# Alibaba-Gemini-Lab/Gemini-SEAL

Measured on AMD Instinct MI355X. Metric: ciphertext multiply+relinearize/s (BFV N=2^15, 8 primes, bit-exact PARITY mode), higher is better.
Workload: dtype u64

## Files before the change

gemini-seal_amd/csrc/devmath.hpp:

```cpp
#pragma once

#include <hip/hip_runtime.h>

#include <cstdint>
#include "ntt_bounds.hpp"
#include "dotacc.hpp"

namespace sealhip
{
    using u64 = unsigned long long;

    struct PrimeDev
    {
        u64 p;
        u64 two_p;
        u64 rdp;
        u64 cr0, cr1;
        u64 inv_n, inv_n_shoup;
        u64 inv_n_w, inv_n_w_shoup;
        u64 ninv;
        const u64 *fwd;
        const u64 *inv;
        const double *fwd_d;
        const double *inv_d;
        double p_d, pinv_d;
    };

    constexpr double kTwo52 = 4503599627370496.0;
    __device__ __forceinline__ double fp_of(u64 bits)
    {
        return __longlong_as_double(static_cast<long long>(bits));
    }
    __device__ __forceinline__ u64 fp_bits(double v)
    {
        return static_cast<u64>(__double_as_longlong(v));
    }
    __device__ __forceinline__ double fp_from_u64(u64 x)
    {
        return fp_of(x | 0x4330000000000000ull) - kTwo52;
    }
    __device__ __forceinline__ u64 fp_to_u64(double r)
    {
        return fp_bits(r + kTwo52) & 0x000FFFFFFFFFFFFFull;
    }
    __device__ __forceinline__ double fp_reduce(double x, double p, double pinv)
    {
#pragma clang fp contract(off)
        return __builtin_fma(-__builtin_rint(x * pinv), p, x);
    }
    __device__ __forceinline__ double fp_canonical(double x, double p, double pinv)
    {
        const double r = fp_reduce(x, p, pinv);
        return r < 0.0 ? r + p : r;
    }
    __device__ __forceinline__ double fp_mulmod(double y, double w, double p, double pinv)
    {
#pragma clang fp contract(off)
        const double h = y * w;
        const double l = __builtin_fma(y, w, -h);
        const double q = __builtin_rint(h * pinv);
        return __builtin_fma(-q, p, h) + l;
    }
    __device__ __forceinline__ void fp_butterfly_fwd(u64 &ub, u64 &yb, u64 wb, double p, double pinv)
    {
        const double u = fp_of(ub), r = fp_mulmod(fp_of(yb), fp_of(wb), p, pinv);
        ub = fp_bits(u + r);
        yb = fp_bits(u - r);
    }
    __device__ __forceinline__ void fp_butterfly_inv(u64 &ub, u64 &yb, u64 wb, double p, double pinv)
    {
        const double u = fp_of(ub), y = fp_of(yb);
        ub = fp_bits(u + y);
        yb = fp_bits(fp_mulmod(u - y, fp_of(wb), p, pinv));
    }

    __device__ __forceinline__ void note_nonzero(unsigned *__restrict__ tflags, std::size_t item, u64 nz)
    {
        if (tflags != nullptr && nz != 0 && tflags[item] == 0)
            tflags[item] = 1;
    }

    __device__ __forceinline__ void store_stream(u64 *p, u64 v)
    {
        __builtin_nontemporal_store(v, p);
    }
    __device__ __forceinline__ void store_stream2(u64 *p, u64 a, u64 b)
    {
        typedef u64 u64x2_s __attribute__((ext_vector_type(2)));
        u64x2_s v;
        v.x = a;
        v.y = b;
        __builtin_nontemporal_store(v, reinterpret_cast<u64x2_s *>(p));
    }

    __device__ __forceinline__ u64 mulhi(u64 a, u64 b)
    {
        return __umul64hi(a, b);
    }

    __device__ __forceinline__ u64 mulmod_lazy(u64 x, u64 y, u64 yshoup, u64 p)
    {
        u64 q = mulhi(x, yshoup);
        return x * y - q * p;
    }

    __device__ __forceinline__ u64 mulmod_shoup(u64 x, u64 y, u64 yshoup, u64 p)
    {
        u64 t = mulmod_lazy(x, y, yshoup, p);
        return t >= p ? t - p : t;
    }

    __device__ __forceinline__ u64 barrett_lazy(u64 x, u64 rdp, u64 p)
    {
        return x - mulhi(x, rdp) * p;
    }

    __device__ __forceinline__ u64 barrett_reduce_128(u64 lo, u64 hi, u64 p, u64 cr0, u64 cr1)
    {
        u64 carry = mulhi(lo, cr0);
        u64 t_lo = lo * cr1, t_hi = mulhi(lo, cr1);
        u64 tmp1 = t_lo + carry;
        u64 tmp3 = t_hi + (tmp1 < t_lo);
        u64 u_lo = hi * cr0, u_hi = mulhi(hi, cr0);
        u64 tmp1b = tmp1 + u_lo;
        u64 carry2 = u_hi + (tmp1b < tmp1);
        u64 q = hi * cr1 + tmp3 + carry2;
        u64 r = lo - q * p;
        return r >= p ? r - p : r;
    }

    __device__ __forceinline__ u64 redc128(u64 lo, u64 hi, u64 p, u64 ninv)
    {
        const u64 m = lo * ninv;
        return hi + mulhi(m, p) + (lo != 0);
    }
    __device__ __forceinline__ u64 redc_finish(u64 t, u64 p, u64 rdp, bool small)
    {
        if (!small)
            t = t - mulhi(t, rdp) * p;
        return t >= p ? t - p : t;
    }

    __device__ __forceinline__ u64 barrett_reduce_63(u64 x, u64 p, u64 cr1)
    {
        u64 r = x - mulhi(x, cr1) * p;
        return r >= p ? r - p : r;
    }

    __device__ __forceinline__ u64 mul_mod(u64 a, u64 b, u64 p, u64 cr0, u64 cr1)
    {
        return barrett_reduce_128(a * b, mulhi(a, b), p, cr0, cr1);
    }

    __device__ __forceinline__ u64 mul_add_mod(u64 a, u64 b, u64 c, u64 p, u64 cr0, u64 cr1)
    {
        u64 lo = a * b, hi = mulhi(a, b);
        u64 lo2 = lo + c;
        hi += (lo2 < lo);
        return barrett_reduce_128(lo2, hi, p, cr0, cr1);
    }

    __device__ __forceinline__ void mac128(u64 &lo, u64 &hi, u64 a, u64 b)
    {
        u64 pl = a * b, ph = mulhi(a, b);
        u64 nl = lo + pl;
        hi += ph + (nl < lo);
        lo = nl;
    }

    __device__ __forceinline__ u64 add_mod(u64 a, u64 b, u64 p)
    {
        u64 s = a + b;
        return s >= p ? s - p : s;
    }
    __device__ __forceinline__ u64 sub_mod(u64 a, u64 b, u64 p)
    {
        u64 d = a - b;
        return a < b ? d + p : d;
// ... 506 lines not shown
```

gemini-seal_amd/csrc/engine.cpp:

```cpp
#include "engine.hpp"

#include <algorithm>
#include <atomic>
#include <cstdlib>
#include <cstring>

namespace sealhip
{
    namespace
    {
        template <class T>
        T *upload(Engine &e, std::vector<void *> &owned, const T *host, std::size_t count)
        {
            T *dev = nullptr;
            SEALHIP_CHECK(hipMalloc(reinterpret_cast<void **>(&dev), sizeof(T) * (count ? count : 1)));
            owned.push_back(dev);
            if (count)
                SEALHIP_CHECK(hipMemcpy(dev, host, sizeof(T) * count, hipMemcpyHostToDevice));
            (void)e;
            return dev;
        }

        RowMap make_map(const std::vector<unsigned short> &ids)
        {
            RowMap m{};
            if (ids.size() > static_cast<std::size_t>(kMaxRows))
                throw std::invalid_argument("too many rows per polynomial");
            m.rows = static_cast<int>(ids.size());
            for (std::size_t i = 0; i < ids.size(); i++)
                m.prime[i] = ids[i];
            return m;
        }
    }

    unsigned long long next_pool_id();

    std::unique_ptr<Engine> make_engine(int scheme, int logn, const u64 *key_moduli, int n_key, int nsp, u64 t,
                                        bool strict, int device)
    {
        if (scheme != 1 && scheme != 2)
            throw std::invalid_argument("unsupported scheme");
        if (logn < 3 || logn > 16)
            throw std::invalid_argument("poly_modulus_degree is invalid");
        if (n_key < 2 || n_key > kMaxModuli || nsp < 1 || n_key <= nsp)
            throw std::invalid_argument("coeff_modulus / n_special_primes invalid");
        if (scheme == 1 && t < 2)
            throw std::invalid_argument("plain_modulus is invalid");
        auto e = std::make_unique<Engine>();
        e->scheme = scheme;
        e->logn = logn;
        e->n = std::size_t(1) << logn;
        e->n_key = n_key;
        e->nsp = nsp;
        e->k_first = n_key - nsp;
        e->t = scheme == 1 ? t : 0;
        e->mode_strict = strict;
        e->use_half_kernel = true;
        e->device = device;
        e->key_moduli.assign(key_moduli, key_moduli + n_key);
        for (int i = 0; i < n_key; i++)
        {
            HostModulus check(e->key_moduli[i]);
            (void)check;
            for (int j = 0; j < i; j++)
                if (e->key_moduli[i] == e->key_moduli[j])
                    throw std::invalid_argument("coeff_modulus primes must be distinct");
        }
        if (scheme == 1)
            e->aux_primes = get_primes(e->n, 60, static_cast<std::size_t>(n_key) + 3);
        const bool batching = scheme == 1 && (t - 1) % (2 * static_cast<u64>(e->n)) == 0 && is_prime_u64(t);
        const int n_primes = n_key + static_cast<int>(e->aux_primes.size()) + (batching ? 1 : 0);
        if (batching)
            e->plain_prime = n_primes - 1;
        e->tables.resize(n_primes);
        for (int i = 0; i < n_primes; i++)
        {
            const u64 p = i == e->plain_prime ? t : i < n_key ? e->key_moduli[i] : e->aux_primes[i - n_key];
            if (i == n_key + 1 && i != e->plain_prime)
            {
                e->tables[i].logn = logn;
                e->tables[i].p = p;
                continue;
            }
            e->tables[i].build(logn, p);
        }
        if (device < 0)
            return e;

        SEALHIP_CHECK(hipSetDevice(device));
        e->lanes = std::make_shared<LanePool>();
        e->lanes->device = device;
        e->lanes->id = next_pool_id();
        SEALHIP_CHECK(ntt_init_kernels());
        std::vector<PrimeDev> pd(n_primes);
        for (int i = 0; i < n_primes; i++)
        {
            const HostNttTables &tb = e->tables[i];
            HostModulus m(tb.p);
            PrimeDev &d = pd[i];
            d.p = tb.p;
            d.two_p = tb.p << 1;
            d.rdp = tb.rdp ? tb.rdp : shoup(1, tb.p);
            d.cr0 = m.cr0;
            d.cr1 = m.cr1;
            d.inv_n = tb.inv_n;
            d.inv_n_shoup = tb.inv_n_shoup;
            d.inv_n_w = tb.inv_n_w;
            d.inv_n_w_shoup = tb.inv_n_w_shoup;
            {
                u64 inv = tb.p;
                for (int it = 0; it < 6; it++)
                    inv *= 2 - tb.p * inv;
                d.ninv = 0 - inv;
            }
            d.fwd = tb.fwd.empty() ? nullptr : upload<u64>(*e, e->owned, tb.fwd.data(), tb.fwd.size());
            d.inv = tb.inv.empty() ? nullptr : upload<u64>(*e, e->owned, tb.inv.data(), tb.inv.size());
            d.fwd_d = d.inv_d = nullptr;
            d.p_d = static_cast<double>(tb.p);
            d.pinv_d = 1.0 / d.p_d;
            if (tb.p < kFpPrimeBound && tb.logn >= 14 && !tb.fwd.empty())
            {
                std::vector<double> f(tb.fwd.size() / 2), v(tb.inv.size() / 2);
                for (std::size_t j = 0; j < f.size(); j++)
                    f[j] = static_cast<double>(tb.fwd[2 * j]);
                for (std::size_t j = 0; j < v.size(); j++)
                    v[j] = static_cast<double>(tb.inv[2 * j]);
                d.fwd_d = upload<double>(*e, e->owned, f.data(), f.size());
                d.inv_d = upload<double>(*e, e->owned, v.data(), v.size());
            }
        }
        e->d_primes = upload<PrimeDev>(*e, e->owned, pd.data(), pd.size());
        return e;
    }

    Lane::~Lane()
    {
        if (device < 0)
            return;
        (void)hipSetDevice(device);
        if (stream)
            (void)hipStreamSynchronize(stream);
        for (ProfRecord &r : prof)
        {
            if (r.start)
                (void)hipEventDestroy(r.start);
            if (r.stop)
                (void)hipEventDestroy(r.stop);
        }
        if (stage)
            free_host_stage(stage);
        if (seed_pin_done)
            (void)hipEventDestroy(seed_pin_done);
        if (seed_pin)
            (void)hipHostFree(seed_pin);
        if (ws)
            (void)hipFree(ws);
        if (d_tickets)
            (void)hipFree(d_tickets);
        if (h_fault)
            (void)hipHostFree(h_fault);
        if (own_stream && stream)
            (void)hipStreamDestroy(stream);
    }

    Lane *LanePool::take()
    {
        std::lock_guard<std::mutex> lock(mu);
        if (!idle.empty())
        {
            Lane *l = idle.back();
            idle.pop_back();
            l->tsink = l->tsink_cur = l->tsink_arm = nullptr;
            l->tsink_cap = l->tsink_base = 0;
            return l;
        }
        auto l = std::make_unique<Lane>();
        l->device = device;
        SEALHIP_CHECK(hipSetDevice(device));
        SEALHIP_CHECK(hipStreamCreateWithFlags(&l->stream, hipStreamNonBlocking));
        l->own_stream = true;
        SEALHIP_CHECK(hipHostMalloc(reinterpret_cast<void **>(&l->h_fault), sizeof(unsigned), hipHostMallocMapped));
        *l->h_fault = 0;
        SEALHIP_CHECK(hipHostGetDevicePointer(reinterpret_cast<void **>(&l->d_fault), l->h_fault, 0));
        all.push_back(std::move(l));
        return all.back().get();
    }

    void LanePool::give(Lane *lane)
    {
        lane->tsink = lane->tsink_cur = lane->tsink_arm = nullptr;
        lane->tsink_cap = lane->tsink_base = 0;
        std::lock_guard<std::mutex> lock(mu);
        idle.push_back(lane);
    }

    namespace
    {
        struct ThreadLanes
        {
            struct Held
            {
                std::weak_ptr<LanePool> pool;
                Lane *lane;
            };
            std::vector<Held> held;
            ~ThreadLanes()
            {
                for (Held &h : held)
                    if (auto p = h.pool.lock())
                        p->give(h.lane);
            }
        };
        thread_local ThreadLanes t_lanes;
        thread_local unsigned long long t_cur_pool_id = 0;
        thread_local Lane *t_cur_lane = nullptr;
        std::atomic<unsigned long long> g_pool_serial{ 0 };
    }

    unsigned long long next_pool_id()
    {
        return ++g_pool_serial;
    }

    Lane &Engine::lane() const
    {
        if (!lanes)
            throw std::logic_error("host-only context: no device");
        if (t_cur_pool_id == lanes->id)
            return *t_cur_lane;
        auto &held = t_lanes.held;
        for (std::size_t i = 0; i < held.size();)
        {
            auto p = held[i].pool.lock();
            if (!p)
            {
                held.erase(held.begin() + static_cast<std::ptrdiff_t>(i));
                continue;
            }
            if (p.get() == lanes.get())
            {
                t_cur_pool_id = lanes->id;
                t_cur_lane = held[i].lane;
                return *t_cur_lane;
            }
            i++;
        }
        Lane *l = lanes->take();
        held.push_back({ lanes, l });
        t_cur_pool_id = lanes->id;
        t_cur_lane = l;
        return *l;
    }

    void Engine::sync_and_check(bool all_lanes) const
    {
        if (all_lanes)
        {
            std::vector<hipStream_t> streams;
            {
                std::lock_guard<std::mutex> lock(lanes->mu);
                for (auto &l : lanes->all)
                    if (!l->capturing)
// ... 790 lines not shown
```

gemini-seal_amd/csrc/engine.hpp:

```cpp
#pragma once

#include <hip/hip_runtime.h>

#include <cstddef>
#include <array>
#include <atomic>
#include <cstdint>
#include <functional>
#include <map>
#include <memory>
#include <mutex>
#include <stdexcept>
#include <string>
#include <cstdlib>
#include <vector>

#include "devmath.hpp"
#include "ntt_bounds.hpp"
#include "hostmath.hpp"

namespace sealhip
{
    constexpr int kMaxRows = 136;
    constexpr int kMaxModuli = 64;
// ... 275 lines not shown
        const std::uint32_t *batch_map();
        mutable std::mutex mu;
        void prof_begin(const char *tag, double units) const;
        void prof_end() const;
        unsigned *ntt_tickets(std::size_t nrows) const;

        ~Engine();
        int n_primes() const
        {
            return static_cast<int>(tables.size());
        }
        LevelTools &level(int k);
        LevelTools &level_host(int k);
        LevelTools &level_rescale(int k);
        const std::uint32_t *galois_table(std::uint32_t elt);
        void ws_reset() const
        {
            Lane &l = lane();
            l.ws_used = l.ws_floor;
        }
        u64 *ws_alloc(std::size_t words) const;
        void ws_reserve(std::size_t bytes) const;
        RowMap map_for(int k, unsigned base);
        int rows_for(int k, unsigned base);
    };

    struct HipError : std::runtime_error
    {
        hipError_t code;
        HipError(hipError_t c, const char *what) : std::runtime_error(what), code(c)
        {}
    };
#define SEALHIP_CHECK(expr)                                                                          \
    do                                                                                               \
    {                                                                                                \
        hipError_t _e = (expr);                                                                      \
        if (_e != hipSuccess)                                                                        \
            throw ::sealhip::HipError(_e, (std::string(#expr) + ": " + hipGetErrorString(_e)).c_str()); \
    } while (0)
    inline void check(hipError_t err, const char *what)
    {
        if (err != hipSuccess)
            throw HipError(err, (std::string(what) + ": " + hipGetErrorString(err)).c_str());
    }

    constexpr int kThreads = 256;
    inline unsigned grid_for(std::size_t work_items, std::size_t max_blocks = 256u * 16u)
    {
        const std::size_t blocks = (work_items + kThreads - 1) / kThreads;
        return static_cast<unsigned>(blocks < max_blocks ? (blocks ? blocks : 1) : max_blocks);
    }

    struct ProfScope
    {
        const Engine &e;
        ProfScope(const Engine &eng, const char *tag, double units) : e(eng)
        {
            if (e.lane().prof_on)
                e.prof_begin(tag, units);
        }
        ~ProfScope()
        {
            if (e.lane().prof_on)
                e.prof_end();
        }
    };

    hipError_t ntt_init_kernels();
    hipError_t ntt_butterfly_rate(const Engine &e, int kind, int prime_id, double *butterflies_per_s);
    hipError_t launch_ntt(const Engine &e, u64 *data, std::size_t nrows, const RowMap &map, bool inverse, int flags);
    bool ntt_can_gather(const Engine &e);
    bool ntt_strict_top_done_ok(const Engine &e, const RowMap &map);
    hipError_t launch_ntt_gather(const Engine &e, u64 *data, std::size_t nrows, const RowMap &map, const NttSource &src,
                                 int flags);

    enum class PolyOp
    {
        Dyadic,
        Add,
        Sub,
        Negate,
        Scalar,
        Mod63
    };
    hipError_t launch_poly_op(const Engine &e, PolyOp op, const u64 *a, const u64 *b, u64 scalar, u64 *r,
                              std::size_t nrows, const RowMap &map);
    hipError_t launch_tensor_product(const Engine &e, const u64 *a, int sa, std::size_t a_stride, const u64 *b, int sb,
                                     std::size_t b_stride, u64 *out, std::size_t out_stride, std::size_t count,
                                     const RowMap &map, bool square = false);
    hipError_t launch_fill_rows(const Engine &e, u64 *dst, const u64 *row_values, int rows, std::size_t count);
    constexpr int kDotGroup = bounds::kDotGroupTerms;
    struct DotTerms
    {
        const u64 *a[kDotGroup];
        const u64 *b[kDotGroup];
        int n;
    };
    hipError_t launch_tensor_dot(const Engine &e, const DotTerms &terms, std::size_t a_stride, std::size_t b_stride, u64 *out01,
                                 std::size_t out01_stride, u64 *out2, std::size_t out2_stride, std::size_t count,
                                 const RowMap &map, bool reduce_on_load, bool add_partial);
    constexpr int kLinGroup = bounds::kLinGroupTerms, kLinTile = bounds::kLinTileSums;
    struct LinTerms
    {
        const u64 *x[kLinGroup];
        int n;
    };
    hipError_t launch_lincomb(const Engine &e, const LinTerms &terms, int size, std::size_t x_stride, const u64 *w,
                              std::size_t w_sum_stride, const u64 *constant, int const_mode, u64 *out, std::size_t out_sum_stride,
                              int n_sums, std::size_t count, const RowMap &map, bool add_partial, std::size_t flag_sum_stride);
    hipError_t launch_poly_tables(const Engine &e, int k, const u64 *coeffs, std::size_t n_coeffs, std::size_t ms, u64 *w,
                                  u64 *constant);
    hipError_t launch_copy_rows(const Engine &e, const u64 *src, std::size_t src_poly_stride, u64 *dst,
                                std::size_t dst_poly_stride, std::size_t npolys, int rows);

    hipError_t launch_fastbconv_m_tilde(const Engine &e, const RnsDev *d, const RnsDev &h, const u64 *in,
                                        std::size_t in_stride, u64 *out, std::size_t out_stride, std::size_t count);
    hipError_t launch_sm_mrq(const Engine &e, const RnsDev *d, const RnsDev &h, const u64 *in, std::size_t in_stride,
                             u64 *out, std::size_t out_stride, std::size_t count);
    constexpr int kBehzGeneric = 32;
    constexpr int kBehzStepwise = 64;
    struct BfvMulPlan
    {
        int k, B, nB;
        bool square;
        bool redc_small;
        bool gather;
        bool defer;
        bool fused_tensor;
        bool tensor_apx;
        bool lift_top;
        int lift_kernel;
        int floor_kernel;
        int deferred_top;
    };
    BfvMulPlan plan_bfv_multiply(Engine &e, int k, int sa, int sb, bool square);

    bool bfv_lift_can_apply_top(const Engine &e, int k, bool redc_small);
    hipError_t launch_bfv_lift(const Engine &e, const RnsDev *d, const RnsDev &h, const u64 *in, std::size_t in_stride,
                               u64 *out, std::size_t out_stride, std::size_t count, const BfvMulPlan &plan);
    hipError_t launch_fast_floor(const Engine &e, const RnsDev *d, const RnsDev &h, const u64 *in,
                                 std::size_t in_stride, u64 *out, std::size_t out_stride, std::size_t count,
                                 int mul_t);
    hipError_t launch_fastbconv_sk(const Engine &e, const RnsDev *d, const RnsDev &h, const u64 *in,
                                   std::size_t in_stride, u64 *out, std::size_t out_stride, std::size_t count);
    hipError_t launch_bfv_floor_sk(const Engine &e, const RnsDev *d, const RnsDev &h, const u64 *in,
                                   std::size_t in_stride, u64 *out, std::size_t out_stride, std::size_t count,
                                   const BfvMulPlan &plan);
    bool ntt_can_defer_top(const Engine &e, int k);
    bool ntt_can_fuse_moddown(const Engine &e, int k, u64 p_special);
    hipError_t launch_intt_from(const Engine &e, u64 *data, const u64 *src, std::size_t src_poly_stride, std::size_t nrows,
                                const RowMap &map, int flags);
    hipError_t launch_intt_tensor(const Engine &e, u64 *data, const u64 *x, std::size_t item_stride, std::size_t poly_stride,
                                  int kb, std::size_t nrows, const RowMap &map, int flags, bool square = false);
    hipError_t launch_divround_bfv(const Engine &e, const RnsDev *d, const RnsDev &h, const u64 *in,
                                   std::size_t in_stride, u64 *out, std::size_t out_stride, std::size_t count,
                                   int out_rows);
    hipError_t launch_rescale_pre(const Engine &e, const RnsDev *d, const RnsDev &h, u64 *last,
                                  std::size_t last_stride, u64 *temp, std::size_t temp_stride, std::size_t count);
    hipError_t launch_rescale_post(const Engine &e, const RnsDev *d, const RnsDev &h, const u64 *in,
                                   std::size_t in_stride, const u64 *temp, std::size_t temp_stride, u64 *out,
                                   std::size_t out_stride, std::size_t count);

    enum class CtLinearOp
    {
        Add,
        Sub,
        Negate,
        MulPlain
    };
    hipError_t launch_ct_linear(const Engine &e, CtLinearOp op, const u64 *a, int sa, const u64 *b, int sb,
                                std::size_t b_item_stride, u64 *out, std::size_t count, const RowMap &map);
    hipError_t launch_nonzero_words(const Engine &e, const u64 *data, std::size_t item_stride, std::size_t words,
                                    std::size_t count, unsigned *flags);
    hipError_t launch_nonzero_tail(const Engine &e, const u64 *ct, std::size_t item_words, std::size_t skip_words,
                                   std::size_t count, unsigned *flags);
    hipError_t launch_out_of_range(const Engine &e, const u64 *ct, std::size_t item_words, std::size_t count,
                                   const RowMap &map, unsigned *flags);
    hipError_t launch_plain_lift(const Engine &e, const u64 *plain, std::size_t plain_stride, u64 *out, std::size_t nplains,
                                 const RowMap &map, u64 t);
    hipError_t launch_plain_lift_centered(const Engine &e, const u64 *plain, std::size_t coeff_count, std::size_t plain_stride,
                                          u64 *out, std::size_t nplains, const RowMap &map, u64 t);
    hipError_t launch_galois(const Engine &e, const u64 *in, u64 *out, std::size_t nrows, const RowMap &map,
                             std::uint32_t elt, const std::uint32_t *table );

    hipError_t launch_ks_modup(const Engine &e, const KsDev *d, const KsDev &h, const u64 *coeff,
                               std::size_t coeff_stride, u64 *ext, std::size_t ext_stride,
                               std::size_t ext_digit_stride, std::size_t count, int only_digit);
    hipError_t launch_ks_mac(const Engine &e, const KsDev *d, const KsDev &h, const u64 *target,
                             std::size_t target_stride, const u64 *ext, std::size_t ext_stride,
                             std::size_t ext_digit_stride, const u64 *key, u64 *prod, std::size_t prod_stride,
                             std::size_t count, int j0 = 0, int j1 = -1);
    hipError_t launch_ks_moddown_pre(const Engine &e, const KsDev *d, const KsDev &h, const u64 *prod,
                                     std::size_t prod_stride, u64 *temp, std::size_t temp_stride, std::size_t npolys);
    hipError_t launch_ks_moddown_bfv(const Engine &e, const KsDev *d, const KsDev &h, const u64 *prod,
                                     std::size_t prod_stride, u64 *ct, std::size_t ct_item_stride, std::size_t npolys,
                                     bool top_deferred, const u64 *c0_src = nullptr, std::size_t c0_stride = 0);
    hipError_t launch_ks_moddown_post(const Engine &e, const KsDev *d, const KsDev &h, u64 *prod,
                                      std::size_t prod_stride, const u64 *temp, std::size_t temp_stride, u64 *ct,
                                      std::size_t ct_item_stride, std::size_t npolys, int add_into_ct,
                                      const u64 *c0_src = nullptr, std::size_t c0_stride = 0);
    hipError_t launch_ks_rescale_fold(const Engine &e, const KsRescaleDev *d, const KsRescaleDev &h, const u64 *base,
                                      std::size_t base_stride, u64 *acc, std::size_t acc_stride, std::size_t npolys);
    hipError_t launch_ks_moddown_rescale_pre(const Engine &e, const KsRescaleDev *d, const KsRescaleDev &h, const u64 *acc,
                                             std::size_t acc_stride, u64 *temp, std::size_t npolys);
    hipError_t launch_ks_moddown_rescale_post(const Engine &e, const KsRescaleDev *d, const KsRescaleDev &h, const u64 *base,
                                              std::size_t base_stride, const u64 *acc, std::size_t acc_stride, const u64 *temp,
                                              u64 *out, std::size_t npolys);

    constexpr int kHoistMaxElts = 16;
    struct HoistElts
    {
        int n;
        std::uint32_t elt[kHoistMaxElts];
        const std::uint32_t *table[kHoistMaxElts];
        const u64 *key[kHoistMaxElts];
    };
    hipError_t launch_hoist_mac(const Engine &e, const KsDev *d, const KsDev &h, const u64 *target,
                                std::size_t target_stride, const u64 *ext, std::size_t ext_stride,
                                std::size_t ext_digit_stride, const HoistElts &elts, u64 *prod, std::size_t prod_stride,
                                std::size_t count);
    hipError_t launch_hoist_galois_c0(const Engine &e, const u64 *ct, std::size_t ct_stride, u64 *out, std::size_t count,
                                      const RowMap &map_q, const HoistElts &elts, bool ntt_form);
    struct HoistDotElts
    {
        int n;
        const std::uint32_t *table[kHoistMaxElts];
        const u64 *key[kHoistMaxElts];
        const u64 *w[kHoistMaxElts];
    };
    hipError_t launch_hoist_dot_mac(const Engine &e, const KsDev *d, const KsDev &h, const u64 *target,
                                    std::size_t target_stride, const u64 *ext, std::size_t ext_stride,
                                    std::size_t ext_digit_stride, const HoistDotElts &elts, std::size_t w_sum_stride, u64 *acc,
                                    std::size_t acc_stride, std::size_t count, std::size_t n_sums, bool add);
    hipError_t launch_hoist_dot_base(const Engine &e, const u64 *cn, const HoistDotElts &elts, std::size_t w_sum_stride,
                                     u64 *out, std::size_t out_sum_stride, int k, std::size_t count, std::size_t n_sums,
                                     bool add);

    struct HoistGiantElts
    {
        int n;
        const std::uint32_t *table[kHoistMaxElts];
        const u64 *key[kHoistMaxElts];
        const u64 *inb[kHoistMaxElts];
        const u64 *ext[kHoistMaxElts];
        const u64 *accj[kHoistMaxElts];
    };
    hipError_t launch_hoist_giant_mac(const Engine &e, const KsDev *d, const KsDev &h, const HoistGiantElts &elts,
                                      std::size_t inb_stride, std::size_t ext_stride, std::size_t ext_digit_stride,
                                      std::size_t accj_stride, u64 *acc, std::size_t acc_stride, std::size_t count, bool add);
    struct HoistGiantBases
    {
        int n;
        const std::uint32_t *table[kHoistMaxElts];
        const u64 *base[kHoistMaxElts];
    };
    hipError_t launch_hoist_giant_base(const Engine &e, const HoistGiantBases &elts, u64 *out, int k, std::size_t count,
                                       bool add);

    struct HostBatchIO
    {
        struct In
        {
            const u64 *const *ptrs;
            std::size_t words;
        };
        struct Out
        {
            u64 *const *ptrs;
            std::size_t words;
        };
        std::vector<In> in;
        std::vector<Out> out;
        std::size_t tmp_words = 0;
    };
    using HostChunkFn = std::function<void(Engine &, const std::vector<u64 *> &d_in, const std::vector<u64 *> &d_out, u64 *d_tmp,
                                           std::size_t m)>;
    void run_host_batch(Engine &e, const HostBatchIO &io, std::size_t count, const HostChunkFn &fn);
    void host_register(const Engine &e, void *ptr, std::size_t bytes);
    void host_unregister(const Engine &e, void *ptr);

    struct KsSplit
    {
        int j0 = 0, j1 = 0;
        u64 *partial_out = nullptr;
        u64 *partial_sum = nullptr;
    };
    void op_switch_key(Engine &e, int k, u64 *ct, std::size_t ct_stride, const u64 *target, std::size_t target_stride,
                       std::size_t count, const KSwitchKey &key, const u64 *c0_src = nullptr, std::size_t c0_stride = 0,
                       const KsSplit *split = nullptr);
    void op_switch_key_rescale(Engine &e, int k, const u64 *base, std::size_t base_stride, const u64 *target,
                               std::size_t target_stride, std::size_t count, const KSwitchKey &key, u64 *out);
    void op_modup(Engine &e, int k, int bundle, u64 *ext, std::size_t count);
    void op_bfv_multiply(Engine &e, int k, const u64 *a, int sa, const u64 *b, int sb, std::size_t count, u64 *out);
    void op_ckks_multiply(Engine &e, int k, const u64 *a, int sa, const u64 *b, int sb, std::size_t count, u64 *out);
    void op_dot_product(Engine &e, int k, const u64 *const *a, const u64 *const *b, std::size_t n_terms, std::size_t count,
                        const KSwitchKey *key, u64 *out, bool rescale = false);
    std::uint64_t dot_product_max_terms(Engine &e, int k);
    void op_linear_combination(Engine &e, int k, const u64 *const *terms, std::size_t n_terms, int size, std::size_t count,
                               const u64 *weights, const u64 *constant, std::size_t n_sums, u64 *out);
    void op_bfv_square(Engine &e, int k, const u64 *a, int sa, std::size_t count, u64 *out);
    void op_ckks_square(Engine &e, int k, const u64 *a, int sa, std::size_t count, u64 *out);
    void op_mod_switch_scale(Engine &e, int k, const u64 *ct, int size, std::size_t count, u64 *out,
                             std::size_t in_item_stride = 0);
    void op_divround_ntt_inplace(Engine &e, int k, u64 *data, std::size_t count);
    void op_rescale_special_inplace(Engine &e, int k, u64 *poly, std::size_t count);
    void op_apply_galois(Engine &e, int k, u64 *ct, std::size_t count, std::uint32_t elt, const KSwitchKey &key);
    void op_apply_galois_many(Engine &e, int k, const u64 *ct, std::size_t count, const std::uint32_t *elts,
                              const KSwitchKey *const *keys, std::size_t n_elts, u64 *out,
                              const std::uint32_t *slots = nullptr);
    void op_apply_galois_dot_plain(Engine &e, int k, const u64 *ct, std::size_t count, const std::uint32_t *elts,
                                   const KSwitchKey *const *keys, std::size_t n_elts, const u64 *plain_ntt,
                                   std::size_t n_sums, u64 *out, bool rescale = false);
    void op_apply_galois_bsgs_plain(Engine &e, int k, const u64 *ct, std::size_t count, const std::uint32_t *baby_elts,
                                    const KSwitchKey *const *baby_keys, std::size_t n_baby, const std::uint32_t *giant_elts,
                                    const KSwitchKey *const *giant_keys, std::size_t n_giant, const u64 *plain_ntt, u64 *out,
                                    bool rescale = false);
    void op_multiply_plain(Engine &e, int k, u64 *ct, int size, std::size_t count, const u64 *plain,
                           std::size_t plain_stride);
    void op_transform_plain_to_ntt(Engine &e, int k, const u64 *plain, std::size_t coeff_count, std::size_t plain_stride,
                                   std::size_t count, u64 *plain_ntt);
    void op_dot_product_ct_sk(Engine &e, int k, const u64 *ct, int size, std::size_t count, const u64 *sk_powers,
                              bool is_ntt_form, u64 *out);
    hipError_t launch_dot_sk(const Engine &e, const u64 *ct, int size, std::size_t ct_item_stride, const u64 *sk_powers,
                             std::size_t sk_power_stride, u64 *out, std::size_t count, const RowMap &map, int add_c0);
    hipError_t launch_decrypt_scale_and_round(const Engine &e, const RnsDev *d, const RnsDev &h, const u64 *in, u64 *out,
                                              std::size_t count);

    struct RlweArgs
    {
        u64 *ct;
        std::size_t ct_item_stride, ct_poly_stride;
        int polys, rows;
        const u64 *x;
        std::size_t x_item_stride, x_poly_stride;
        const u64 *y;
        std::size_t y_poly_stride;
        const std::int32_t *e;
        std::size_t e_item_stride, e_poly_stride;
        int negate;
    };
    struct ScalingArgs
    {
        const u64 *plain;
        std::size_t plain_item_stride;
        u64 *c0;
        std::size_t c0_item_stride;
        int k, sub;
        u64 t, t_cr0, t_cr1, q_mod_t, threshold;
        u64 div[kMaxModuli];
// ... 107 lines not shown
```

gemini-seal_amd/csrc/keyswitch.hip:

```cpp
#include <cstdlib>
#include "engine.hpp"

namespace sealhip
{
    namespace
    {
        __device__ __forceinline__ const u64 *modup_block(const KsDev *d, int j)
        {
            const int rows = d->k + d->nsp;
            return d->modup + static_cast<std::size_t>(j) * (2 * d->nsp + rows * d->nsp);
        }

        __global__ __launch_bounds__(kThreads) void ks_modup_kernel(const KsDev *__restrict__ d,
                                                                    const PrimeDev *__restrict__ primes,
                                                                    const u64 *__restrict__ coeff,
                                                                    std::size_t coeff_stride, u64 *__restrict__ ext,
                                                                    std::size_t ext_stride,
                                                                    std::size_t ext_digit_stride, std::size_t count,
                                                                    int logn, int only_digit)
        {
            const std::size_t i = blockIdx.x * static_cast<std::size_t>(blockDim.x) + threadIdx.x;
            const std::size_t item = i >> logn;
            if (item >= count)
                return;
// ... 100 lines not shown
            u64 *pp = prod + item * prod_stride + static_cast<std::size_t>(r) * N + c;
            pp[0] = barrett_reduce_128(lo0, hi0, P.p, P.cr0, P.cr1);
            pp[static_cast<std::size_t>(rows) * N] = barrett_reduce_128(lo1, hi1, P.p, P.cr0, P.cr1);
        }

        template <int ND>
        __global__ __launch_bounds__(kThreads) void ks_mac_items_kernel(const KsDev *__restrict__ d,
                                                                        const PrimeDev *__restrict__ primes,
                                                                        const u64 *__restrict__ target,
                                                                        std::size_t target_stride,
                                                                        const u64 *__restrict__ ext,
                                                                        std::size_t ext_stride,
                                                                        std::size_t ext_digit_stride,
                                                                        const u64 *__restrict__ key,
                                                                        u64 *__restrict__ prod, std::size_t prod_stride,
                                                                        std::size_t count, int logn, std::size_t group)
        {
            const std::size_t N = static_cast<std::size_t>(1) << logn;
            const int k = d->k, nsp = d->nsp, rows = k + nsp, n_total = d->n_total;
            const std::size_t i = blockIdx.x * static_cast<std::size_t>(blockDim.x) + threadIdx.x;
            const std::size_t c = i & (N - 1);
            const std::size_t rr = i >> logn;
            const int r = static_cast<int>(rr % rows);
            const std::size_t item0 = (rr / rows) * group;
            if (item0 >= count)
                return;
            const std::size_t item1 = item0 + group < count ? item0 + group : count;
            const int rns_idx = d->row_prime[r];
            const int my_digit = r < k ? r / nsp : -1;
            const std::size_t row_off = static_cast<std::size_t>(r) * N + c;
            const u64 *pkey = key + static_cast<std::size_t>(rns_idx) * N + c;
            const std::size_t key_comp = static_cast<std::size_t>(n_total) * N;
            u64 k0[ND], k1[ND], x[ND], xn[ND];
#pragma unroll
            for (int j = 0; j < ND; j++)
            {
                k0[j] = pkey[(2 * static_cast<std::size_t>(j)) * key_comp];
                k1[j] = pkey[(2 * static_cast<std::size_t>(j) + 1) * key_comp];
            }
            auto load_x = [&](u64(&dst)[ND], std::size_t item) {
#pragma unroll
                for (int j = 0; j < ND; j++)
                    dst[j] = j == my_digit ? target[item * target_stride + row_off]
                                           : ext[item * ext_stride + static_cast<std::size_t>(j) * ext_digit_stride + row_off];
            };
            load_x(x, item0);
            const PrimeDev &P = primes[rns_idx];
            const u64 p = P.p, cr0 = P.cr0, cr1 = P.cr1;
            for (std::size_t item = item0; item < item1; item++)
            {
                if (item + 1 < item1)
                    load_x(xn, item + 1);
                u64 lo0 = 0, hi0 = 0, lo1 = 0, hi1 = 0;
#pragma unroll
                for (int j = 0; j < ND; j++)
                {
                    mac128(lo0, hi0, x[j], k0[j]);
                    mac128(lo1, hi1, x[j], k1[j]);
                }
                u64 *pp = prod + item * prod_stride + row_off;
                store_stream(pp, barrett_reduce_128(lo0, hi0, p, cr0, cr1));
                store_stream(pp + static_cast<std::size_t>(rows) * N, barrett_reduce_128(lo1, hi1, p, cr0, cr1));
#pragma unroll
                for (int j = 0; j < ND; j++)
                    x[j] = xn[j];
            }
        }

        __global__ __launch_bounds__(kThreads) void ks_moddown_pre_kernel(const KsDev *__restrict__ d,
                                                                          const PrimeDev *__restrict__ primes,
                                                                          const u64 *__restrict__ prod,
                                                                          std::size_t prod_stride,
                                                                          u64 *__restrict__ temp,
                                                                          std::size_t temp_stride, std::size_t npolys,
                                                                          int logn)
        {
            const std::size_t i = blockIdx.x * static_cast<std::size_t>(blockDim.x) + threadIdx.x;
            const std::size_t poly = i >> logn;
            if (poly >= npolys)
                return;
            const std::size_t N = static_cast<std::size_t>(1) << logn;
            const std::size_t c = i & (N - 1);
            const int k = d->k, nsp = d->nsp;
            const u64 *sp = prod + poly * prod_stride + static_cast<std::size_t>(k) * N + c;
            u64 *pt = temp + poly * temp_stride + c;
            if (nsp == 1)
            {
                const PrimeDev &S = primes[d->row_prime[k]];
                const u64 v = neg_mod(barrett_reduce_63(sp[0], S.p, S.cr1), S.p);
                for (int q = 0; q < k; q++)
                {
                    const PrimeDev &Q = primes[d->row_prime[q]];
                    pt[q * N] = barrett_reduce_63(v, Q.p, Q.cr1);
                }
                return;
            }
            for (int q = 0; q < k; q++)
            {
                const PrimeDev &Q = primes[d->row_prime[q]];
                u64 lo = 0, hi = 0;
                for (int j = 0; j < nsp; j++)
                {
                    const u64 pj = primes[d->row_prime[k + j]].p;
                    const u64 y = mulmod_shoup(sp[j * N], d->inv_hat[j], d->inv_hat_shoup[j], pj);
                    mac128(lo, hi, y, d->neg_hat[q * nsp + j]);
                }
                pt[q * N] = barrett_reduce_128(lo, hi, Q.p, Q.cr0, Q.cr1);
            }
        }

        __global__ __launch_bounds__(kThreads) void ks_moddown_post_kernel(const KsDev *__restrict__ d,
                                                                           const PrimeDev *__restrict__ primes,
                                                                           u64 *__restrict__ prod,
                                                                           std::size_t prod_stride,
                                                                           const u64 *__restrict__ temp,
                                                                           std::size_t temp_stride,
                                                                           u64 *__restrict__ ct,
                                                                           std::size_t ct_item_stride,
                                                                           std::size_t npolys, int logn,
                                                                           int add_into_ct, const u64 *__restrict__ c0_src,
                                                                           std::size_t c0_stride, unsigned *__restrict__ tflags)
        {
            const std::size_t N = static_cast<std::size_t>(1) << logn;
            const int k = d->k;
            const std::size_t i = blockIdx.x * static_cast<std::size_t>(blockDim.x) + threadIdx.x;
            const std::size_t c = i & (N - 1);
            const std::size_t rr = i >> logn;
            const int q = static_cast<int>(rr % k);
            const std::size_t poly = rr / k;
            if (poly >= npolys)
                return;
            const PrimeDev &Q = primes[d->row_prime[q]];
            u64 *pp = prod + poly * prod_stride + static_cast<std::size_t>(q) * N + c;
            const u64 v = mulmod_shoup(*pp + temp[poly * temp_stride + static_cast<std::size_t>(q) * N + c], d->invP[q],
                                       d->invP_shoup[q], Q.p);
            if (add_into_ct)
            {
                u64 *pc = ct + (poly >> 1) * ct_item_stride + ((poly & 1) * static_cast<std::size_t>(k) + q) * N + c;
                u64 w;
                if (!c0_src)
                    w = add_mod(v, *pc, Q.p);
                else
                    w = (poly & 1) ? v : add_mod(v, c0_src[(poly >> 1) * c0_stride + static_cast<std::size_t>(q) * N + c], Q.p);
                *pc = w;
                if (poly & 1)
                    note_nonzero(tflags, poly >> 1, w);
            }
            else
                *pp = v;
        }

        template <bool DEFER>
        __device__ __forceinline__ void row_pair(const u64 *__restrict__ row, std::size_t c_lo, std::size_t half,
                                                 const PrimeDev &P, u64 &x_lo, u64 &x_hi)
        {
            const u64 u = row[c_lo], v = row[c_lo + half];
            if (!DEFER)
            {
                x_lo = u;
                x_hi = v;
                return;
            }
            u64 tt = u + v;
            tt = tt >= P.two_p ? tt - P.two_p : tt;
            x_lo = mulmod_lazy(tt, P.inv_n, P.inv_n_shoup, P.p);
            x_hi = mulmod_lazy(u - v + P.two_p, P.inv_n_w, P.inv_n_w_shoup, P.p);
        }

        template <bool DEFER, bool ONE>
        __global__ __launch_bounds__(kThreads) void ks_moddown_bfv_kernel(const KsDev *__restrict__ d,
                                                                          const PrimeDev *__restrict__ primes,
                                                                          const u64 *__restrict__ prod,
                                                                          std::size_t prod_stride, u64 *__restrict__ ct,
                                                                          std::size_t ct_item_stride, std::size_t npolys,
                                                                          int logn, const u64 *__restrict__ c0_src,
                                                                          std::size_t c0_stride, unsigned *__restrict__ tflags)
        {
            const std::size_t N = static_cast<std::size_t>(1) << logn, half = N >> 1;
            const int k = d->k, nsp = d->nsp;
            const std::size_t i = blockIdx.x * static_cast<std::size_t>(blockDim.x) + threadIdx.x;
            const std::size_t c = i & (half - 1);
            const std::size_t poly = i >> (logn - 1);
            if (poly >= npolys)
                return;
            const u64 *pp = prod + poly * prod_stride;
            u64 sred[2] = {0, 0};
            if constexpr (ONE)
            {
                const PrimeDev &S = primes[d->row_prime[k]];
                u64 sv[2];
                row_pair<DEFER>(pp + static_cast<std::size_t>(k) * N, c, half, S, sv[0], sv[1]);
#pragma unroll
                for (int h = 0; h < 2; h++)
                    sred[h] = neg_mod(barrett_reduce_63(sv[h], S.p, S.cr1), S.p);
            }
            u64 nz = 0;
            for (int q = 0; q < k; q++)
            {
                const PrimeDev &Q = primes[d->row_prime[q]];
                u64 temp[2];
                if constexpr (ONE)
                {
#pragma unroll
                    for (int h = 0; h < 2; h++)
                        temp[h] = barrett_reduce_63(sred[h], Q.p, Q.cr1);
                }
                else
                {
                    u64 lo[2] = {0, 0}, hi[2] = {0, 0};
                    for (int j = 0; j < nsp; j++)
                    {
                        const PrimeDev &S = primes[d->row_prime[k + j]];
                        u64 sv[2];
                        row_pair<DEFER>(pp + static_cast<std::size_t>(k + j) * N, c, half, S, sv[0], sv[1]);
#pragma unroll
                        for (int h = 0; h < 2; h++)
                        {
                            const u64 y = mulmod_shoup(sv[h], d->inv_hat[j], d->inv_hat_shoup[j], S.p);
                            mac128(lo[h], hi[h], y, d->neg_hat[q * nsp + j]);
                        }
                    }
                    temp[0] = barrett_reduce_128(lo[0], hi[0], Q.p, Q.cr0, Q.cr1);
                    temp[1] = barrett_reduce_128(lo[1], hi[1], Q.p, Q.cr0, Q.cr1);
                }
                u64 pv[2];
                row_pair<DEFER>(pp + static_cast<std::size_t>(q) * N, c, half, Q, pv[0], pv[1]);
                u64 *pc = ct + (poly >> 1) * ct_item_stride + ((poly & 1) * static_cast<std::size_t>(k) + q) * N + c;
#pragma unroll
                for (int h = 0; h < 2; h++)
                {
                    const u64 v = mulmod_shoup(pv[h] + temp[h], d->invP[q], d->invP_shoup[q], Q.p);
                    u64 w;
                    if (!c0_src)
                        w = add_mod(v, pc[h * half], Q.p);
                    else
                        w = (poly & 1) ? v
                                       : add_mod(v, c0_src[(poly >> 1) * c0_stride + static_cast<std::size_t>(q) * N + c + h * half], Q.p);
                    pc[h * half] = w;
                    nz |= w;
                }
            }
            if (poly & 1)
                note_nonzero(tflags, poly >> 1, nz);
        }

        __global__ __launch_bounds__(kThreads) void ks_rescale_fold_kernel(const KsRescaleDev *__restrict__ d,
                                                                           const PrimeDev *__restrict__ primes,
                                                                           const u64 *__restrict__ base, std::size_t base_stride,
                                                                           u64 *__restrict__ acc, std::size_t acc_stride,
                                                                           std::size_t npolys, int logn)
        {
            const std::size_t i = blockIdx.x * static_cast<std::size_t>(blockDim.x) + threadIdx.x;
            const std::size_t poly = i >> logn;
            if (poly >= npolys)
                return;
            const std::size_t N = static_cast<std::size_t>(1) << logn;
            const std::size_t c = i & (N - 1);
            const int k = d->k;
            const PrimeDev &L = primes[d->drop_prime[0]];
            const u64 b = base[(poly >> 1) * base_stride + ((poly & 1) * static_cast<std::size_t>(k) + (k - 1)) * N + c];
            u64 *pa = acc + poly * acc_stride + static_cast<std::size_t>(k - 1) * N + c;
            *pa = mul_add_mod(b, d->P_mod_l, *pa, L.p, L.cr0, L.cr1);
        }

        __device__ __forceinline__ u64 rescale_z(const KsRescaleDev *__restrict__ d, const PrimeDev *__restrict__ primes, int a,
                                                 u64 y, u64 &slo, u64 &shi)
        {
            const PrimeDev &S = primes[d->drop_prime[a]];
            const u64 z = mulmod_shoup(add_mod(y, d->half_d[a], S.p), d->inv_hat[a], d->inv_hat_shoup[a], S.p);
            const u64 t = z * S.cr1 + mulhi(z, S.cr0);
            const u64 nl = slo + t;
            shi += nl < slo;
            slo = nl;
            return z;
        }

        template <int ND1>
        __global__ __launch_bounds__(kThreads) void ks_moddown_rescale_pre_kernel(const KsRescaleDev *__restrict__ d,
                                                                                  const PrimeDev *__restrict__ primes,
                                                                                  const u64 *__restrict__ acc,
                                                                                  std::size_t acc_stride, u64 *__restrict__ temp,
                                                                                  std::size_t npolys, int logn)
        {
            const std::size_t i = blockIdx.x * static_cast<std::size_t>(blockDim.x) + threadIdx.x;
            const std::size_t poly = i >> logn;
            if (poly >= npolys)
                return;
            const std::size_t N = static_cast<std::size_t>(1) << logn;
            const std::size_t c = i & (N - 1);
            const int k = d->k, nd1 = d->nsp + 1;
            const u64 *dp = acc + poly * acc_stride + static_cast<std::size_t>(k - 1) * N + c;
            u64 *pt = temp + poly * static_cast<std::size_t>(k - 1) * N + c;
            u64 slo = 0, shi = 0;
            if constexpr (ND1 > 0)
            {
                u64 z[ND1];
#pragma unroll
                for (int a = 0; a < ND1; a++)
                    z[a] = rescale_z(d, primes, a, dp[a * N], slo, shi);
                const u64 v = shi;
                for (int r = 0; r < k - 1; r++)
                {
                    const PrimeDev &Q = primes[r];
                    const u64 *hat = d->hat + static_cast<std::size_t>(r) * ND1;
                    u64 lo = d->neg_half[r], hi = 0;
#pragma unroll
                    for (int a = 0; a < ND1; a++)
                        mac128(lo, hi, z[a], hat[a]);
                    mac128(lo, hi, v, d->neg_D[r]);
                    pt[r * N] = barrett_reduce_128(lo, hi, Q.p, Q.cr0, Q.cr1);
                }
            }
            else
            {
                for (int a = 0; a < nd1; a++)
                    rescale_z(d, primes, a, dp[a * N], slo, shi);
                const u64 v = shi;
                for (int r = 0; r < k - 1; r++)
                {
                    const PrimeDev &Q = primes[r];
                    const u64 *hat = d->hat + static_cast<std::size_t>(r) * nd1;
                    u64 lo = d->neg_half[r], hi = 0, s0 = 0, s1 = 0;
                    for (int a = 0; a < nd1; a++)
                        mac128(lo, hi, rescale_z(d, primes, a, dp[a * N], s0, s1), hat[a]);
                    mac128(lo, hi, v, d->neg_D[r]);
                    pt[r * N] = barrett_reduce_128(lo, hi, Q.p, Q.cr0, Q.cr1);
                }
            }
        }

        __global__ __launch_bounds__(kThreads) void ks_moddown_rescale_post_kernel(const KsRescaleDev *__restrict__ d,
                                                                                   const PrimeDev *__restrict__ primes,
                                                                                   const u64 *__restrict__ base,
                                                                                   std::size_t base_stride,
                                                                                   const u64 *__restrict__ acc,
                                                                                   std::size_t acc_stride,
                                                                                   const u64 *__restrict__ temp, u64 *__restrict__ out,
                                                                                   std::size_t npolys, int logn,
                                                                                   unsigned *__restrict__ tflags)
        {
            const std::size_t N = static_cast<std::size_t>(1) << logn;
            const int k = d->k, kk = k - 1;
            const std::size_t i = blockIdx.x * static_cast<std::size_t>(blockDim.x) + threadIdx.x;
            const std::size_t c = i & (N - 1);
            const std::size_t rr = i >> logn;
            const int r = static_cast<int>(rr % kk);
            const std::size_t poly = rr / kk;
            if (poly >= npolys)
                return;
            const PrimeDev &Q = primes[r];
            const std::size_t row = static_cast<std::size_t>(r) * N + c;
            const u64 b = base[(poly >> 1) * base_stride + (poly & 1) * static_cast<std::size_t>(k) * N + row];
            const u64 s = mul_add_mod(b, d->P_mod_q[r], acc[poly * acc_stride + row], Q.p, Q.cr0, Q.cr1);
            const std::size_t o = poly * static_cast<std::size_t>(kk) * N + row;
            const u64 w = mulmod_shoup(sub_mod(s, temp[o], Q.p), d->invD[r], d->invD_shoup[r], Q.p);
            store_stream(out + o, w);
            if (poly & 1)
                note_nonzero(tflags, poly >> 1, w);
        }

        inline unsigned blocks_for(std::size_t lanes)
        {
            return static_cast<unsigned>((lanes + kThreads - 1) / kThreads);
        }
    }

    hipError_t launch_ks_modup(const Engine &e, const KsDev *d, const KsDev &, const u64 *coeff,
                               std::size_t coeff_stride, u64 *ext, std::size_t ext_stride,
                               std::size_t ext_digit_stride, std::size_t count, int only_digit)
    {
        if (!count)
            return hipSuccess;
        ProfScope prof(e, "ks_modup", 0);
        ks_modup_kernel<<<blocks_for(count << e.logn), kThreads, 0, e.lane().stream>>>(
            d, e.d_primes, coeff, coeff_stride, ext, ext_stride, ext_digit_stride, count, e.logn, only_digit);
        return hipGetLastError();
    }

    hipError_t launch_ks_mac(const Engine &e, const KsDev *d, const KsDev &h, const u64 *target,
                             std::size_t target_stride, const u64 *ext, std::size_t ext_stride,
                             std::size_t ext_digit_stride, const u64 *key, u64 *prod, std::size_t prod_stride,
                             std::size_t count, int j0, int j1)
    {
        if (!count)
            return hipSuccess;
        if (j1 < 0)
            j1 = h.nd;
        if (j0 < 0 || j0 > j1 || j1 > h.nd)
            return hipErrorInvalidValue;
        const bool all_digits = j0 == 0 && j1 == h.nd;
        const u64 *tg = target;
        const std::size_t lanes = (count * static_cast<std::size_t>(h.k + h.nsp)) << e.logn;
        ProfScope prof(e, "ks_mac", 0);
        const std::size_t key_bytes = (2ull * h.nd * (h.k + h.nsp)) << (e.logn + 3);
        const std::size_t cap = key_bytes > (std::size_t(48) << 20) ? 64 : 16;
        std::size_t mac_group = 8;
        for (std::size_t g = cap; g > 8; g >>= 1)
            if ((((count + g - 1) / g * static_cast<std::size_t>(h.k + h.nsp)) << e.logn) / kThreads >= 4096)
            {
                mac_group = g;
                break;
            }
        const std::size_t groups = (count + mac_group - 1) / mac_group;
        const std::size_t glanes = (groups * static_cast<std::size_t>(h.k + h.nsp)) << e.logn;
#define SEALHIP_KS_MAC(ND)                                                                                          \
    case ND:                                                                                                        \
        ks_mac_items_kernel<ND><<<blocks_for(glanes), kThreads, 0, e.lane().stream>>>(                                     \
            d, e.d_primes, tg, target_stride, ext, ext_stride, ext_digit_stride, key, prod, prod_stride, count,    \
            e.logn, mac_group);                                                                                     \
        break;
        switch (count >= 16 && all_digits ? h.nd : 0)
        {
            SEALHIP_KS_MAC(1)
            SEALHIP_KS_MAC(2)
            SEALHIP_KS_MAC(3)
            SEALHIP_KS_MAC(4)
            SEALHIP_KS_MAC(5)
            SEALHIP_KS_MAC(6)
            SEALHIP_KS_MAC(7)
            SEALHIP_KS_MAC(8)
            SEALHIP_KS_MAC(9)
            SEALHIP_KS_MAC(10)
            SEALHIP_KS_MAC(11)
            SEALHIP_KS_MAC(12)
            SEALHIP_KS_MAC(13)
            SEALHIP_KS_MAC(14)
            SEALHIP_KS_MAC(15)
            SEALHIP_KS_MAC(16)
        default:
            ks_mac_kernel<<<blocks_for(lanes), kThreads, 0, e.lane().stream>>>(d, e.d_primes, tg, target_stride, ext, ext_stride,
                                                                        ext_digit_stride, key, prod, prod_stride, count,
                                                                        e.logn, j0, j1);
        }
#undef SEALHIP_KS_MAC
        return hipGetLastError();
    }

    hipError_t launch_ks_moddown_pre(const Engine &e, const KsDev *d, const KsDev &, const u64 *prod,
                                     std::size_t prod_stride, u64 *temp, std::size_t temp_stride, std::size_t npolys)
    {
        if (!npolys)
            return hipSuccess;
        ProfScope prof(e, "ks_moddown_pre", 0);
        ks_moddown_pre_kernel<<<blocks_for(npolys << e.logn), kThreads, 0, e.lane().stream>>>(
            d, e.d_primes, prod, prod_stride, temp, temp_stride, npolys, e.logn);
        return hipGetLastError();
    }

    hipError_t launch_ks_moddown_bfv(const Engine &e, const KsDev *d, const KsDev &h, const u64 *prod,
                                     std::size_t prod_stride, u64 *ct, std::size_t ct_item_stride, std::size_t npolys,
                                     bool top_deferred, const u64 *c0_src, std::size_t c0_stride)
    {
        if (!npolys)
            return hipSuccess;
        const std::size_t lanes = npolys << (e.logn - 1);
        ProfScope prof(e, "ks_moddown_bfv", 0);
#define SEALHIP_MODDOWN_BFV(DEFER_, ONE_)                                                                            \
    ks_moddown_bfv_kernel<DEFER_, ONE_><<<blocks_for(lanes), kThreads, 0, e.lane().stream>>>(                              \
        d, e.d_primes, prod, prod_stride, ct, ct_item_stride, npolys, e.logn, c0_src, c0_stride, e.lane().tsink_arm)
        if (top_deferred && h.nsp == 1)
            SEALHIP_MODDOWN_BFV(true, true);
        else if (top_deferred)
            SEALHIP_MODDOWN_BFV(true, false);
        else if (h.nsp == 1)
            SEALHIP_MODDOWN_BFV(false, true);
        else
            SEALHIP_MODDOWN_BFV(false, false);
#undef SEALHIP_MODDOWN_BFV
        return hipGetLastError();
    }

    hipError_t launch_ks_moddown_post(const Engine &e, const KsDev *d, const KsDev &h, u64 *prod,
                                      std::size_t prod_stride, const u64 *temp, std::size_t temp_stride, u64 *ct,
                                      std::size_t ct_item_stride, std::size_t npolys, int add_into_ct, const u64 *c0_src,
                                      std::size_t c0_stride)
    {
        if (!npolys)
            return hipSuccess;
        const std::size_t lanes = (npolys * static_cast<std::size_t>(h.k)) << e.logn;
        ProfScope prof(e, "ks_moddown_post", 0);
        ks_moddown_post_kernel<<<blocks_for(lanes), kThreads, 0, e.lane().stream>>>(
            d, e.d_primes, prod, prod_stride, temp, temp_stride, ct, ct_item_stride, npolys, e.logn, add_into_ct, c0_src, c0_stride,
            add_into_ct ? e.lane().tsink_arm : nullptr);
        return hipGetLastError();
    }

    hipError_t launch_ks_rescale_fold(const Engine &e, const KsRescaleDev *d, const KsRescaleDev &, const u64 *base,
                                      std::size_t base_stride, u64 *acc, std::size_t acc_stride, std::size_t npolys)
    {
        if (!npolys)
            return hipSuccess;
        ProfScope prof(e, "ks_rescale_fold", 0);
        ks_rescale_fold_kernel<<<blocks_for(npolys << e.logn), kThreads, 0, e.lane().stream>>>(d, e.d_primes, base, base_stride, acc,
                                                                                            acc_stride, npolys, e.logn);
        return hipGetLastError();
    }

    hipError_t launch_ks_moddown_rescale_pre(const Engine &e, const KsRescaleDev *d, const KsRescaleDev &h, const u64 *acc,
                                             std::size_t acc_stride, u64 *temp, std::size_t npolys)
    {
        if (!npolys)
            return hipSuccess;
        ProfScope prof(e, "ks_moddown_rescale_pre", 0);
#define SEALHIP_RESCALE_PRE(ND1)                                                                                     \
    ks_moddown_rescale_pre_kernel<ND1><<<blocks_for(npolys << e.logn), kThreads, 0, e.lane().stream>>>(                    \
        d, e.d_primes, acc, acc_stride, temp, npolys, e.logn)
        switch (h.nsp + 1)
        {
        case 2:
            SEALHIP_RESCALE_PRE(2);
            break;
        case 3:
            SEALHIP_RESCALE_PRE(3);
            break;
        case 4:
            SEALHIP_RESCALE_PRE(4);
            break;
        default:
            SEALHIP_RESCALE_PRE(0);
        }
#undef SEALHIP_RESCALE_PRE
        return hipGetLastError();
    }

    hipError_t launch_ks_moddown_rescale_post(const Engine &e, const KsRescaleDev *d, const KsRescaleDev &h, const u64 *base,
                                              std::size_t base_stride, const u64 *acc, std::size_t acc_stride, const u64 *temp,
                                              u64 *out, std::size_t npolys)
    {
        if (!npolys)
            return hipSuccess;
        const std::size_t lanes = (npolys * static_cast<std::size_t>(h.k - 1)) << e.logn;
        ProfScope prof(e, "ks_moddown_rescale_post", 0);
        ks_moddown_rescale_post_kernel<<<blocks_for(lanes), kThreads, 0, e.lane().stream>>>(
            d, e.d_primes, base, base_stride, acc, acc_stride, temp, out, npolys, e.logn, e.lane().tsink_arm);
        return hipGetLastError();
    }
}
```

gemini-seal_amd/csrc/ntt.hip:

```cpp
#include <cstdlib>
#include <stdexcept>

#include "ntt_half.hpp"

namespace sealhip
{
    namespace
    {
        constexpr int kTileBitsMax = 13;

        __device__ __forceinline__ int pad_index(int l)
        {
            return l + (l >> 4);
        }

        template <int DIR>
        __global__ __launch_bounds__(512, 4) void ntt_pass_kernel(u64 *__restrict__ data,
                                                               const PrimeDev *__restrict__ primes, RowMap map,
                                                               NttPass ps)
        {
            extern __shared__ u64 lds[];
            const int tid = threadIdx.x;
            const int nthreads = blockDim.x;
            const int t = ps.t, c = ps.c, b_lo = ps.b_lo, logn = ps.logn;
// ... 378 lines not shown
                    if ((it & 1) == 1)
                    {
#pragma unroll
                        for (int i = 0; i < 16; i++)
                            x[i] = fp_bits(fp_reduce(fp_of(x[i]), fp_of(two_p), fp_of(neg_p)));
                    }
            }
            u64 acc = 0;
#pragma unroll
            for (int i = 0; i < 16; i++)
                acc ^= x[i];
            if (acc == 0x0123456789ABCDEFull)
                sink[0] = acc;
        }
    }

    hipError_t ntt_butterfly_rate(const Engine &e, int kind, int prime_id, double *butterflies_per_s)
    {
        if (kind < 0 || kind > 5 || prime_id < 0 || prime_id >= static_cast<int>(e.tables.size()))
            return hipErrorInvalidValue;
        PrimeDev P{};
        hipError_t err = hipMemcpy(&P, e.d_primes + prime_id, sizeof(P), hipMemcpyDeviceToHost);
        if (err != hipSuccess)
            return err;
        if (kind == 3 && P.fwd_d == nullptr)
            return hipErrorInvalidValue;
        u64 *sink = nullptr;
        if ((err = hipMalloc(&sink, 8)) != hipSuccess)
            return err;
        hipStream_t st = e.lane().stream;
        hipEvent_t a, b;
        (void)hipEventCreate(&a);
        (void)hipEventCreate(&b);
        const unsigned blocks = 256u * 2u * 4u;
        const int iters = 800;
        const std::size_t lds = static_cast<std::size_t>(hpad(1 << 13)) * 8;
        const void *fns[6] = { reinterpret_cast<const void *>(&butterfly_rate_kernel<0>), reinterpret_cast<const void *>(&butterfly_rate_kernel<1>),
                               reinterpret_cast<const void *>(&butterfly_rate_kernel<2>), reinterpret_cast<const void *>(&butterfly_rate_kernel<3>),
                               reinterpret_cast<const void *>(&butterfly_rate_kernel<4>), reinterpret_cast<const void *>(&butterfly_rate_kernel<5>) };
        if ((err = hipFuncSetAttribute(fns[kind], hipFuncAttributeMaxDynamicSharedMemorySize, static_cast<int>(lds))) != hipSuccess)
        {
            (void)hipEventDestroy(a);
            (void)hipEventDestroy(b);
            (void)hipFree(sink);
            return err;
        }
        const auto launch = [&](int n) {
            switch (kind)
            {
            case 0: butterfly_rate_kernel<0><<<blocks, 512, lds, st>>>(sink, P, n); break;
            case 1: butterfly_rate_kernel<1><<<blocks, 512, lds, st>>>(sink, P, n); break;
            case 2: butterfly_rate_kernel<2><<<blocks, 512, lds, st>>>(sink, P, n); break;
            case 3: butterfly_rate_kernel<3><<<blocks, 512, lds, st>>>(sink, P, n); break;
            case 4: butterfly_rate_kernel<4><<<blocks, 512, lds, st>>>(sink, P, n); break;
            default: butterfly_rate_kernel<5><<<blocks, 512, lds, st>>>(sink, P, n); break;
            }
        };
        launch(iters / 8);
        (void)hipEventRecord(a, st);
        launch(iters);
        launch(iters);
        (void)hipEventRecord(b, st);
        err = hipStreamSynchronize(st);
        float ms = 0;
        if (err == hipSuccess)
            err = hipEventElapsedTime(&ms, a, b);
        (void)hipEventDestroy(a);
        (void)hipEventDestroy(b);
        (void)hipFree(sink);
        if (err != hipSuccess)
            return err;
        *butterflies_per_s = 2.0 * blocks * 512.0 * iters * 32.0 / (ms / 1e3);
        return hipGetLastError();
    }

    hipError_t ntt_init_kernels()
    {
        const int max_lds = ((1 << kTileBitsMax) + (1 << (kTileBitsMax - 4))) * 8;
        hipError_t err = hipFuncSetAttribute(reinterpret_cast<const void *>(&ntt_pass_kernel<0>),
                                             hipFuncAttributeMaxDynamicSharedMemorySize, max_lds);
        if (err != hipSuccess)
            return err;
        err = hipFuncSetAttribute(reinterpret_cast<const void *>(&ntt_pass_kernel<1>),
                                  hipFuncAttributeMaxDynamicSharedMemorySize, max_lds);
        if (err == hipSuccess)
            err = ntt_fwd_half_init();
        if (err == hipSuccess)
            err = ntt_inv_half_init();
        return err;
    }

    bool ntt_can_defer_top(const Engine &e, int k)
    {
        return e.use_half_kernel && e.logn >= 14 && e.logn <= 16 && k <= 32;
    }

    bool ntt_can_fuse_moddown(const Engine &e, int k, u64 p_special)
    {
        if (!fp64_enabled() || !ntt_can_gather(e) || e.logn < 15 || p_special >= kFpPrimeBound)
            return false;
        for (int r = 0; r < k; r++)
            if (e.key_moduli[r] >= kFpPrimeBound)
                return false;
        return true;
    }

    bool ntt_strict_top_done_ok(const Engine &e, const RowMap &map)
    {
        if (!e.use_half_kernel || e.logn < 14 || e.logn > 16 || exact_fwd())
            return false;
        for (int r = 0; r < map.rows; r++)
            if (map.prime[r] != kSkipRow && !bounds::fwd_dense_admits(e.tables[map.prime[r]].p, e.logn))
                return false;
        return true;
    }

    bool ntt_can_gather(const Engine &e)
    {
        return e.use_half_kernel && e.logn >= 14 && e.logn <= 16;
    }

    hipError_t launch_ntt_gather(const Engine &e, u64 *data, size_t nrows, const RowMap &map, const NttSource &src,
                                 int flags)
    {
        if (!ntt_can_gather(e))
            return hipErrorInvalidValue;
        if (e.mode_strict)
            flags |= kNttStrict;
        if (nrows == 0)
            return hipSuccess;
        return ntt_fwd_half(e, data, nrows, map, flags, src);
    }

    hipError_t launch_intt_from(const Engine &e, u64 *data, const u64 *src, std::size_t src_poly_stride, size_t nrows,
                                const RowMap &map, int flags)
    {
        if (!(e.use_half_kernel && e.logn >= 14 && e.logn <= 16))
            return hipErrorInvalidValue;
        if (nrows == 0)
            return hipSuccess;
        return ntt_inv_half(e, data, nrows, map, flags, src, src_poly_stride);
    }

    hipError_t launch_intt_tensor(const Engine &e, u64 *data, const u64 *x, std::size_t item_stride, std::size_t poly_stride,
                                  int kb, size_t nrows, const RowMap &map, int flags, bool square)
    {
        if (!(e.use_half_kernel && e.logn >= 14 && e.logn <= 16) || map.rows != 3 * kb)
            return hipErrorInvalidValue;
        if (nrows == 0)
            return hipSuccess;
        return ntt_inv_tensor(e, data, nrows, map, flags, x, item_stride, poly_stride, kb, square);
    }

    hipError_t launch_ntt(const Engine &e, u64 *data, size_t nrows, const RowMap &map, bool inverse, int flags)
    {
        if (nrows == 0)
            return hipSuccess;
        if (e.mode_strict)
            flags |= kNttStrict;
        if (e.use_half_kernel && e.logn >= 14 && e.logn <= 16)
            return inverse ? ntt_inv_half(e, data, nrows, map, flags) : ntt_fwd_half(e, data, nrows, map, flags, NttSource{});
        if (e.logn > kTileBitsMax)
            return hipErrorInvalidValue;
        const NttPlan plan = plan_ntt(e.logn, inverse, flags);
        return inverse ? launch_dir<1>(e, data, nrows, map, plan) : launch_dir<0>(e, data, nrows, map, plan);
    }
}
```

gemini-seal_amd/csrc/ntt_bounds.hpp:

```cpp
#pragma once
#include <cstdint>

namespace sealhip
{
    namespace bounds
    {
        using u64 = unsigned long long;
        using u128 = unsigned __int128;

        constexpr int kMinHalfLogn = 14, kMaxHalfLogn = 16;
        constexpr int kMaxPrimeBits = 61;
        constexpr u128 kWord = static_cast<u128>(1) << 64;
        constexpr long double kFpLimit = 9007199254740992.0L;

        constexpr u64 max_prime_of_bits(int bits)
        {
            return (bits >= 64 ? ~u64(0) : (u64(1) << bits) - 1);
        }
        constexpr u64 max_ntt_prime_of_bits(int bits, int logn)
        {
            return bits > logn + 1 ? (u64(1) << bits) - (u64(1) << (logn + 1)) + 1 : 0;
        }

        constexpr int kInvLazyProductMult = 4;
// ... 204 lines not shown
            }
            return peak;
        }
        constexpr bool fp_inv_reduce_after_layer(int T, int l)
        {
            return l % 4 == 1 && l != T - 1;
        }
        constexpr long double fp_inv_peak(int T, long double p)
        {
            long double b = 2.0L * p, peak = b;
            for (int l = 0; l < T; l++)
            {
                const long double s = 2.0L * b;
                peak = s > peak ? s : peak;
                const long double r = fp_mul_bound(s, p);
                b = s > r ? s : r;
                if (fp_inv_reduce_after_layer(T, l))
                    b = fp_reduce_bound(b, p);
            }
            return peak;
        }
        constexpr int fp_prime_bits()
        {
            int bits = 0;
            for (int b = kMaxHalfLogn + 2; b <= 52; b++)
            {
                bool ok = true;
                for (int logn = kMinHalfLogn; logn <= kMaxHalfLogn; logn++)
                {
                    const long double p = static_cast<long double>(max_ntt_prime_of_bits(b, logn));
                    ok = ok && fp_fwd_peak(logn, p, 0x1p52L) < kFpLimit;
                    ok = ok && fp_inv_peak(logn - 1, p) < kFpLimit;
                    if (logn <= 15)
                        ok = ok && fp_inv_peak(logn, p) < kFpLimit;
                }
                if (ok)
                    bits = b;
            }
            return bits;
        }
        constexpr int kFpPrimeBits = fp_prime_bits();
        static_assert(kFpPrimeBits == 50, "FP64 instances: primes below 2^50 (and raw inputs below 2^52)");
        constexpr u64 kFpInputBound = u64(1) << 52;
        constexpr bool fp_admits(u64 p)
        {
            return p <= max_prime_of_bits(kFpPrimeBits);
        }
        constexpr bool dotacc_ok(int nterms, int bits)
        {
            if (nterms < 1 || bits < 33 || bits > 64)
                return false;
            const u128 lim = kWord;
            const int nm = (2 * nterms + 7) / 8;
            const int per_m = (2 * nterms + nm - 1) / nm;
            const u128 low = static_cast<u128>(nterms) << 48;
            const u128 mid = static_cast<u128>(per_m) << bits;
            const u128 high = static_cast<u128>(nterms) << (2 * (bits - 32));
            return low <= lim && mid <= lim && high <= lim;
        }
        constexpr int kDotAccOperandBits = 61;
        constexpr int dotacc_max_terms()
        {
            int n = 0;
            for (int t = 1; t <= 4096; t++)
                if (dotacc_ok(t, kDotAccOperandBits))
                    n = t;
                else
                    break;
            return n;
        }
        static_assert(dotacc_max_terms() >= 64, "DotAcc on 61-bit operands: at least 64 terms (the kernels use up to k + 2 <= 34)");
        constexpr int dotacc31_nl(int nterms) { return (nterms + 3) / 4; }
        constexpr int dotacc31_nm(int nterms) { return (2 * nterms + 7) / 8; }
        constexpr int dotacc31_nh(int nterms) { return (nterms + 15) / 16; }
        constexpr bool dotacc31_ok(int nterms, int bits)
        {
            if (nterms < 1 || nterms > 64 || bits < 32 || bits > 62)
                return false;
            const u128 lim = kWord;
            const int nl = dotacc31_nl(nterms), nm = dotacc31_nm(nterms), nh = dotacc31_nh(nterms);
            const u128 low = static_cast<u128>((nterms + nl - 1) / nl) << 62;
            const u128 mid = static_cast<u128>((2 * nterms + nm - 1) / nm) << bits;
            const u128 high = static_cast<u128>((nterms + nh - 1) / nh) << (2 * (bits - 31));
            const bool sum_fits = 2 * bits + 6 <= 128;
            return low <= lim && mid <= lim && high <= lim && sum_fits;
        }
        constexpr bool dotacc31_all_ok(int max_terms)
        {
            for (int t = 1; t <= max_terms; t++)
                if (!dotacc31_ok(t, kDotAccOperandBits))
                    return false;
            return true;
        }

        constexpr bool small_quot_admits(u64 p, int mult)
        {
            if (p < kSmallQuotMinPrime || mult < 1 || mult > 128 || static_cast<u128>(mult) * p > kWord)
                return false;
            const long double loss = 0x1p32L / static_cast<long double>(p) +
                                     static_cast<long double>(mult) * (0x1p-20L + 3 * 0x1p-24L + 0x1p-51L);
            return loss <= 0.5L;
        }

        constexpr bool behz_redc_small(int k, int B, u64 max_q, u64 max_b)
        {
            const u128 s1 = static_cast<u128>(k) * max_q + 2 * static_cast<u128>(max_b);
            const u128 s2 = static_cast<u128>(B + 1) * max_b;
            return k >= 1 && B >= 1 && s1 <= kWord && s2 <= kWord;
        }
        static_assert(!behz_redc_small(15, 16, u64(1) << 40, (u64(1) << 60) - (u64(1) << 55)),
                      "s2 at |B| = 16 for every m_sk");
        constexpr int kBehzExactMaxK = 15;
        static_assert(dotacc31_all_ok(kBehzExactMaxK + 2),
                      "DotAcc31 on 61-bit operands: every term count of the exact-k instances (up to k + 2)");

        constexpr bool dot_group_admits(int terms, int bits)
        {
            if (terms < 1 || bits < 1 || bits > 63)
                return false;
            const int shift = 128 - bits;
            if (shift <= bits)
                return false;
            return (static_cast<u128>(2 * terms) << bits) + 1 <= (static_cast<u128>(1) << shift);
        }
        constexpr int kDotGroupTerms = 16;
        static_assert(dot_group_admits(kDotGroupTerms, kDotAccOperandBits), "16 terms of 61-bit operands fit 128 bits");
        static_assert(dot_group_admits(31, kDotAccOperandBits) && !dot_group_admits(32, kDotAccOperandBits),
                      "this (conservative) count admits 31 terms at 61 bits: the group of 16 leaves almost a factor two");
        constexpr bool lincomb_group_admits(int terms, int bits)
        {
            if (terms < 1 || bits < 1 || bits > 63)
                return false;
            const int shift = 128 - bits;
            if (shift <= bits)
                return false;
            return (static_cast<u128>(terms) << bits) + 2 <= (static_cast<u128>(1) << shift);
        }
        constexpr int kLinGroupTerms = 16;
        constexpr int kLinTileSums = 4;
        static_assert(lincomb_group_admits(kLinGroupTerms, kDotAccOperandBits), "16 products of 61-bit words fit 128 bits");
        static_assert(lincomb_group_admits(63, kDotAccOperandBits) && !lincomb_group_admits(64, kDotAccOperandBits),
                      "this (conservative) count admits 63 terms at 61 bits: the group of 16 leaves almost a factor four");

        constexpr bool ks_rescale_sum_fits(int dropped, int bits)
        {
            if (dropped < 1 || bits < 1 || bits > 63)
                return false;
            const u128 m = (static_cast<u128>(1) << bits) - 1, max = ~static_cast<u128>(0);
            const u128 tail = static_cast<u128>(dropped + 1) * m;
            return static_cast<u128>(dropped) <= (max - tail) / (m * m);
        }
        static_assert(ks_rescale_sum_fits(64, kDotAccOperandBits) && !ks_rescale_sum_fits(65, kDotAccOperandBits),
                      "the last prime and up to 63 special primes of 61 bits: 64 dropped primes fit, 65 would not");
    }
}
```

gemini-seal_amd/csrc/ntt_half.hpp:

```cpp
#pragma once
#include "engine.hpp"

#define SEALHIP_INTERNAL __attribute__((visibility("hidden")))

namespace sealhip
{
    SEALHIP_INTERNAL bool fp64_enabled();
    SEALHIP_INTERNAL bool exact_fwd();

    SEALHIP_INTERNAL hipError_t ntt_fwd_half(const Engine &e, u64 *data, std::size_t nrows, const RowMap &map, int flags,
                                             const NttSource &src);
    SEALHIP_INTERNAL hipError_t ntt_inv_half(const Engine &e, u64 *data, std::size_t nrows, const RowMap &map, int flags,
                                             const u64 *src = nullptr, std::size_t src_poly_stride = 0);
    SEALHIP_INTERNAL hipError_t ntt_inv_tensor(const Engine &e, u64 *data, std::size_t nrows, const RowMap &map, int flags,
                                               const u64 *x, std::size_t item_stride, std::size_t poly_stride, int kb,
                                               bool square);
    SEALHIP_INTERNAL hipError_t ntt_fwd_half_init();
    SEALHIP_INTERNAL hipError_t ntt_inv_half_init();

    namespace
    {
        template <int T, int R>
        struct Arr
        {
            static_assert(T >= 13 && T <= 15, "half-row shapes of N = 2^14 .. 2^16: 2^(T-5) lanes, i.e. 2^(T-11) waves <-> index bits [11, T)");
            static constexpr int beta = R <= 3 ? T - 4 * R : 0;
            static constexpr int f = T - 12;
            static constexpr int slot_bit(int w)
            {
                if (w == 0)
                    return 0;
                if (R <= 3)
                    return beta + (w - 1);
                if (w < f)
                    return w;
                return f + 6 + (w - f);
            }
            static constexpr int low_start = R <= 3 ? 1 : f;
            static constexpr int low_len = R <= 3 ? beta - 1 : T - 5;
            static constexpr int high_start = beta + 4;
            __device__ static __forceinline__ int tid_index(int tid)
            {
                if constexpr (R == 4)
                    return ((tid & 63) << f) | ((tid >> 6) << 11);
                int v = (tid & ((1 << low_len) - 1)) << low_start;
                if (R <= 3 && low_len < T - 5)
                    v |= (tid >> low_len) << high_start;
                return v;
            }
            static constexpr bool wave_owned = R == 2 || R == 3 || R == 4;
            static constexpr int slot_index(int s)
            {
                int r = 0;
                for (int w = 0; w < 5; w++)
                    if ((s >> w) & 1)
                        r |= 1 << slot_bit(w);
                return r;
            }
            static constexpr int tw_offset(int s, int w)
            {
                int r = 0;
                for (int v = w + 1; v < 5; v++)
                    if ((s >> v) & 1)
                        r |= 1 << (slot_bit(v) - slot_bit(w) - 1);
                return r;
            }
        };

        typedef u64 u64x2_nt __attribute__((ext_vector_type(2)));
        __device__ __forceinline__ void store_nt(u64 *p, u64 a, u64 b)
        {
            u64x2_nt v;
            v.x = a;
            v.y = b;
            __builtin_nontemporal_store(v, reinterpret_cast<u64x2_nt *>(p));
        }

        __host__ __device__ constexpr int hpad(int e)
        {
            return e + 2 * (e >> 5) + ((e >> 4) & 1);
        }

        template <int T, int RA, int RB>
        __device__ __forceinline__ void h_exchange(u64 (&x)[32], u64 *lds, int tid)
        {
            const int pa = hpad(Arr<T, RA>::tid_index(tid) >> 1);
            const int pb = hpad(Arr<T, RB>::tid_index(tid) >> 1);
            constexpr bool LOCAL = Arr<T, RA>::wave_owned && Arr<T, RB>::wave_owned;
            const auto sync = [] {
                if constexpr (LOCAL)
                {
                    __builtin_amdgcn_fence(__ATOMIC_RELEASE, "wavefront");
                    __builtin_amdgcn_wave_barrier();
                    __builtin_amdgcn_fence(__ATOMIC_ACQUIRE, "wavefront");
                }
                else
                    __syncthreads();
            };
#pragma unroll
            for (int phase = 0; phase < 2; phase++)
            {
#pragma unroll
                for (int s = 0; s < 32; s++)
                    if ((s & 1) == phase)
                        lds[pa + hpad(Arr<T, RA>::slot_index(s) >> 1)] = x[s];
                sync();
#pragma unroll
                for (int s = 0; s < 32; s++)
                    if ((s & 1) == phase)
                        x[s] = lds[pb + hpad(Arr<T, RB>::slot_index(s) >> 1)];
                sync();
            }
        }

        typedef u64 u64x2 __attribute__((ext_vector_type(2)));
        typedef const __attribute__((address_space(1))) u64x2 *tw_global_t;
        typedef const __attribute__((address_space(4))) u64x2 *tw_const_t;
        typedef const __attribute__((address_space(1))) u64 *twd_global_t;
        typedef const __attribute__((address_space(4))) u64 *twd_const_t;
        __device__ __forceinline__ void fp_reduce_all(u64 (&x)[32], u64 p_bits, u64 pinv_bits)
        {
            const double p = fp_of(p_bits), pinv = fp_of(pinv_bits);
#pragma unroll
            for (int i = 0; i < 32; i++)
                x[i] = fp_bits(fp_reduce(fp_of(x[i]), p, pinv));
        }
        constexpr int kIL = 4;
        using ZeroPairs = ZeroHi<2>;

        template <int T>
        struct FinalStage
        {
            static constexpr int f = T - 12;
            static constexpr int NTW = (1 << f) - 1;
            static constexpr int SG = f == 1 ? 4 : (f == 2 ? 2 : 1);
            static constexpr int NG = 1 << (5 - f);
            static constexpr int NS = NG / SG;
            static constexpr bool PIPE = f <= 2;
        };

        struct LiveSlots
        {
            int n;
            unsigned short slot[kMaxRows];
        };
        inline LiveSlots live_slots(const RowMap &map)
        {
            LiveSlots ls{};
            for (int r = 0; r < map.rows; r++)
                if (map.prime[r] != kSkipRow)
                    ls.slot[ls.n++] = static_cast<unsigned short>(r);
            return ls;
        }
        __device__ __forceinline__ bool half_block_map(unsigned bid, std::size_t npolys, int n_live, std::size_t chunk,
                                                       std::size_t &poly, int &position, int &half, int poly_major = 0)
        {
            const unsigned xcd = bid & 7u;
            const std::size_t slot = bid >> 3;
            half = static_cast<int>(slot & 1);
            const std::size_t v = static_cast<std::size_t>(xcd) * chunk + (slot >> 1);
            if ((slot >> 1) >= chunk || v >= npolys * static_cast<std::size_t>(n_live))
                return false;
            if (poly_major)
            {
                const int g = poly_major;
                const std::size_t full = static_cast<std::size_t>(n_live / g) * npolys * g;
                if (v < full)
                {
                    const std::size_t gp = v / g;
// ... 56 lines not shown
```

gemini-seal_amd/csrc/ntt_inv.hip:

```cpp
#include <cstdlib>

#include "ntt_half.hpp"

namespace sealhip
{
    namespace
    {
        template <int LZ>
        constexpr bool kLazy = LZ == 1 || LZ == 3;
        template <int T, int LZ = 1>
        struct InvLazy
        {
            static constexpr int sched = LZ == 3 ? 1 : 0;
            static constexpr int mode(int l)
            {
                return bounds::inv_lazy_mode(T, l, sched);
            }
            static constexpr int shift(int l)
            {
                return bounds::inv_lazy_shift(T, l, sched);
            }
            static constexpr int reduce_mode = LZ == 3 ? 3 : 2;
        };
        template <int KLOGN>
// ... 58 lines not shown
                            x[slot(j)] = fp_bits(fp_reduce(fp_of(x[slot(j)]), pd, pinv));
                            x[slot(j) | bit] = fp_bits(fp_reduce(fp_of(x[slot(j) | bit]), pd, pinv));
                        }
                    }
                    return;
                }
                u64 u[kIL], y[kIL];
#pragma unroll
                for (int j = 0; j < kIL; j++)
                {
                    u[j] = x[slot(j)];
                    y[j] = x[slot(j) | bit];
                }
                if constexpr (kLazy<LZ> && InvLazy<T, LZ>::mode(layer) == 1)
                    butterflies_inv_apx2<UNIFORM, kIL>(u, y, w, ws, neg_p, lazy_addend(neg_p, InvLazy<T, LZ>::shift(layer)), zp.z);
                else if constexpr (kLazy<LZ>)
                    butterflies_inv_hs<UNIFORM, kIL, InvLazy<T, LZ>::mode(layer) == 1 ? 1 : InvLazy<T, LZ>::reduce_mode>(
                        u, y, w, ws, neg_p, lazy_addend(neg_p, InvLazy<T, LZ>::shift(layer)), rdp);
                else
                    butterflies_inv_hs<UNIFORM, kIL>(u, y, w, ws, neg_p, two_p);
#pragma unroll
                for (int j = 0; j < kIL; j++)
                {
                    x[slot(j)] = u[j];
                    x[slot(j) | bit] = y[j];
                }
            }
        };
        template <int T, int R, bool UNIFORM, int LZ, int K = 0, int NLAYERS = 4>
        struct RoundPipeInv
        {
            static constexpr int NST = NLAYERS * (16 / kIL);
            __device__ static __forceinline__ void run(u64 (&x)[32], const u64 (&w)[kIL], const u64 (&ws)[kIL],
                                                       const u64 *__restrict__ tw, int jb, int N, u64 two_p, u64 neg_p,
                                                       u64 rdp, ZeroPairs &zp)
            {
                u64 wn[kIL], wsn[kIL];
                if constexpr (K + 1 < NST)
                    RoundStageInv<T, R, UNIFORM, K + 1, LZ>::load(wn, wsn, tw, jb, N);
                __builtin_amdgcn_sched_barrier(0);
                RoundStageInv<T, R, UNIFORM, K, LZ>::run(x, w, ws, two_p, neg_p, rdp, zp);
                if constexpr (K + 1 < NST)
                    RoundPipeInv<T, R, UNIFORM, LZ, K + 1, NLAYERS>::run(x, wn, wsn, tw, jb, N, two_p, neg_p, rdp, zp);
            }
        };

        template <int T, int G, bool FP = false>
        __device__ __forceinline__ void h_first_tw(u64x2 *tg, const u64 *__restrict__ tw, int jb, int N)
        {
            constexpr int f = T - 12;
            int base = 0;
#pragma unroll
            for (int W = 0; W < f; W++)
            {
                const int tb = (N + jb) >> (Arr<T, 4>::slot_bit(W) + 1);
#pragma unroll
                for (int o = 0; o < (1 << (f - 1 - W)); o++)
                {
                    const int s = (G << f) | (o << (W + 1));
                    if constexpr (FP)
                        tg[base + o].x = ((twd_global_t)tw)[tb + Arr<T, 4>::tw_offset(s, W)];
                    else
                        tg[base + o] = ((tw_global_t)tw)[tb + Arr<T, 4>::tw_offset(s, W)];
                }
                base += 1 << (f - 1 - W);
            }
        }
        template <int T, int G, int LZ>
        __device__ __forceinline__ void h_first_group_regs(u64 (&x)[32], const u64x2 *tg, u64 neg_p, u64 two_p, u64 rdp, ZeroPairs &zp)
        {
            constexpr int f = T - 12;
            static_assert(LZ != 1 || f - 1 < bounds::inv_lazy_r1(T), "sparse schedule: the first layers are never the reducing ones");
            int base = 0;
#pragma unroll
            for (int W = 0; W < f; W++)
            {
                const int bit = 1 << W;
                const u64 addend = kLazy<LZ> ? lazy_addend(neg_p, InvLazy<T, LZ>::shift(W)) : two_p;
#pragma unroll
                for (int e = 0; e < (1 << f); e++)
                {
                    if (e & bit)
                        continue;
                    const int s = (G << f) | e;
                    const u64x2 Wv = tg[base + (e >> (W + 1))];
                    if constexpr (LZ == 2)
                    {
                        const double pd = fp_of(two_p), pinv = fp_of(neg_p);
                        fp_butterfly_inv(x[s], x[s | bit], Wv.x, pd, pinv);
                        if (fp_inv_reduce_after<T>(W))
                        {
                            x[s] = fp_bits(fp_reduce(fp_of(x[s]), pd, pinv));
                            x[s | bit] = fp_bits(fp_reduce(fp_of(x[s | bit]), pd, pinv));
                        }
                        continue;
                    }
                    const u64 u = x[s], v = x[s | bit];
                    u64 tt = u + v;
                    if (!kLazy<LZ>)
                        tt = tt >= two_p ? tt - two_p : tt;
                    else if (InvLazy<T, LZ>::mode(W) != 1)
                        tt = reduce_small_quot(tt, __uint_as_float(static_cast<unsigned>(rdp)), neg_p);
                    x[s] = tt;
                    if (LZ == 1 && InvLazy<T, 1>::mode(W) == 1)
                        x[s | bit] = mulmod_lazy_apx2<false>(u - v + addend, Wv.x, Wv.y, neg_p, zp.z[(e >> (W + 1)) & 1]);
                    else
                        x[s | bit] = mulmod_lazy_hs<false>(u - v + addend, Wv.x, Wv.y, neg_p);
                }
                base += 1 << (f - 1 - W);
            }
        }
        template <int T, int ST, int LZ, int I = 0>
        struct FirstStage
        {
            __device__ static __forceinline__ void load(u64x2 *tg, const u64 *__restrict__ tw, int jb, int N)
            {
                h_first_tw<T, ST * FinalStage<T>::SG + I, LZ == 2>(tg + I * FinalStage<T>::NTW, tw, jb, N);
                if constexpr (I + 1 < FinalStage<T>::SG)
                    FirstStage<T, ST, LZ, I + 1>::load(tg, tw, jb, N);
            }
            __device__ static __forceinline__ void run(u64 (&x)[32], const u64x2 *tg, u64 neg_p, u64 two_p, u64 rdp, ZeroPairs &zp)
            {
                h_first_group_regs<T, ST * FinalStage<T>::SG + I, LZ>(x, tg + I * FinalStage<T>::NTW, neg_p, two_p, rdp, zp);
                if constexpr (I + 1 < FinalStage<T>::SG)
                    FirstStage<T, ST, LZ, I + 1>::run(x, tg, neg_p, two_p, rdp, zp);
            }
        };
        template <int T, int ST, int LZ, bool AHEAD = FinalStage<T>::PIPE>
        struct FirstPipe
        {
            __device__ static __forceinline__ void run(u64 (&x)[32], const u64x2 *cur, const u64 *__restrict__ tw, int jb,
                                                       int N, u64 neg_p, u64 two_p, u64 rdp, ZeroPairs &zp)
            {
                u64x2 next[FinalStage<T>::SG * FinalStage<T>::NTW];
                if constexpr (ST + 1 < FinalStage<T>::NS && AHEAD)
                    FirstStage<T, ST + 1, LZ>::load(next, tw, jb, N);
                __builtin_amdgcn_sched_barrier(0);
                FirstStage<T, ST, LZ>::run(x, cur, neg_p, two_p, rdp, zp);
                __builtin_amdgcn_sched_barrier(0);
                if constexpr (ST + 1 < FinalStage<T>::NS && !AHEAD)
                    FirstStage<T, ST + 1, LZ>::load(next, tw, jb, N);
                if constexpr (ST + 1 < FinalStage<T>::NS)
                    FirstPipe<T, ST + 1, LZ, AHEAD>::run(x, next, tw, jb, N, neg_p, two_p, rdp, zp);
            }
        };

        struct DyadicSrc
        {
            const u64 *x;
            std::size_t item_stride, poly_stride;
            int kb;
            int square;
        };
        template <int IL, int NP>
        __device__ __forceinline__ void dyadic_redc(u64 (&t)[IL], const u64 (&a)[NP][IL], const u64 (&b)[NP][IL], u64 p, u64 ninv)
        {
            static_assert(IL >= 3, "the carry of the high product is read IL instructions after its producer");
            typedef unsigned __int128 u128;
            u64 P0[NP][IL], M[IL], H[IL], cy[IL] = {};
#pragma unroll
            for (int q = 0; q < NP; q++)
            {
#pragma unroll
                for (int j = 0; j < IL; j++)
                    P0[q][j] = mul64v<false>(static_cast<u32>(a[q][j]), static_cast<u32>(b[q][j]), cy[j]);
#pragma unroll
                for (int j = 0; j < IL; j++)
                    M[j] = q == 0 ? mul64v<false>(static_cast<u32>(a[q][j]), static_cast<u32>(b[q][j] >> 32), cy[j])
                                  : mad64v<false>(static_cast<u32>(a[q][j]), static_cast<u32>(b[q][j] >> 32), M[j], cy[j]);
#pragma unroll
                for (int j = 0; j < IL; j++)
                    M[j] = mad64v<false>(static_cast<u32>(a[q][j] >> 32), static_cast<u32>(b[q][j]), M[j], cy[j]);
#pragma unroll
                for (int j = 0; j < IL; j++)
                    H[j] = q == 0 ? mul64v<false>(static_cast<u32>(a[q][j] >> 32), static_cast<u32>(b[q][j] >> 32), cy[j])
                                  : mad64v<false>(static_cast<u32>(a[q][j] >> 32), static_cast<u32>(b[q][j] >> 32), H[j], cy[j]);
            }
            u64 lo[IL], hi[IL], m[IL], A[IL], B[IL], carry[IL], mh[IL];
            u32 cb[IL];
            const u32 p0 = static_cast<u32>(p), p1 = static_cast<u32>(p >> 32);
#pragma unroll
            for (int j = 0; j < IL; j++)
            {
                u128 X = (static_cast<u128>(H[j]) << 64) + (static_cast<u128>(M[j]) << 32);
#pragma unroll
                for (int q = 0; q < NP; q++)
                    X += P0[q][j];
                lo[j] = static_cast<u64>(X);
                hi[j] = static_cast<u64>(X >> 64);
                m[j] = lo[j] * ninv;
            }
#pragma unroll
            for (int j = 0; j < IL; j++)
                A[j] = mad64v<true>(static_cast<u32>(m[j] >> 32), p0, static_cast<u64>(__umulhi(static_cast<u32>(m[j]), p0)), cy[j]);
#pragma unroll
            for (int j = 0; j < IL; j++)
                asm volatile("v_mad_u64_u32 %0, %1, %2, %3, %4" : "=v"(B[j]), "=s"(carry[j]) : "v"(static_cast<u32>(m[j])), "s"(p1), "v"(A[j]));
#pragma unroll
            for (int j = 0; j < IL; j++)
                asm volatile("v_cndmask_b32_e64 %0, 0, 1, %1" : "=v"(cb[j]) : "s"(carry[j]));
#pragma unroll
            for (int j = 0; j < IL; j++)
                mh[j] = mad64v<true>(static_cast<u32>(m[j] >> 32), p1,
                                     static_cast<u64>(static_cast<u32>(B[j] >> 32)) | (static_cast<u64>(cb[j]) << 32), cy[j]);
#pragma unroll
            for (int j = 0; j < IL; j++)
                t[j] = hi[j] + mh[j] + (lo[j] != 0);
        }

        template <int T, bool SAME = false, bool TWICE = false>
        __device__ __forceinline__ void h_load_dyadic2(u64 (&x)[32], const u64 *__restrict__ a, const u64 *__restrict__ b,
                                                       int jloc, u64 p, u64 ninv)
        {
#pragma unroll
            for (int batch = 0; batch < 4; batch++)
            {
                ulonglong2 va[4], vb[4];
#pragma unroll
                for (int i = 0; i < 4; i++)
                {
                    const int idx = jloc + Arr<T, 4>::slot_index((batch * 4 + i) * 2);
                    va[i] = *reinterpret_cast<const ulonglong2 *>(a + idx);
                    if constexpr (SAME)
                        vb[i] = va[i];
                    else
                        vb[i] = *reinterpret_cast<const ulonglong2 *>(b + idx);
                }
#pragma unroll
                for (int g = 0; g < 2; g++)
                {
                    const u64 aa[1][4] = { { va[2 * g].x, va[2 * g].y, va[2 * g + 1].x, va[2 * g + 1].y } };
                    const u64 bb[1][4] = { { vb[2 * g].x, vb[2 * g].y, vb[2 * g + 1].x, vb[2 * g + 1].y } };
                    u64 t[4];
                    dyadic_redc<4, 1>(t, aa, bb, p, ninv);
#pragma unroll
                    for (int j = 0; j < 4; j++)
                    {
                        if constexpr (TWICE)
                        {
                            const u64 d = t[j] << 1, two_p = p << 1;
                            t[j] = d >= two_p ? d - two_p : d;
                        }
                        x[(batch * 4 + 2 * g) * 2 + j] = t[j];
                    }
                }
                __builtin_amdgcn_sched_barrier(0);
            }
        }
        template <int T>
        __device__ __forceinline__ void h_load_dyadic4(u64 (&x)[32], const u64 *__restrict__ a0, const u64 *__restrict__ b1,
                                                       const u64 *__restrict__ a1, const u64 *__restrict__ b0, int jloc, u64 p,
                                                       u64 ninv)
        {
#pragma unroll
            for (int batch = 0; batch < 8; batch++)
            {
                ulonglong2 v0[2], v1[2], v2[2], v3[2];
#pragma unroll
                for (int i = 0; i < 2; i++)
                {
                    const int idx = jloc + Arr<T, 4>::slot_index((batch * 2 + i) * 2);
                    v0[i] = *reinterpret_cast<const ulonglong2 *>(a0 + idx);
                    v1[i] = *reinterpret_cast<const ulonglong2 *>(b1 + idx);
                    v2[i] = *reinterpret_cast<const ulonglong2 *>(a1 + idx);
                    v3[i] = *reinterpret_cast<const ulonglong2 *>(b0 + idx);
                }
                const u64 aa[2][4] = { { v0[0].x, v0[0].y, v0[1].x, v0[1].y }, { v2[0].x, v2[0].y, v2[1].x, v2[1].y } };
                const u64 bb[2][4] = { { v1[0].x, v1[0].y, v1[1].x, v1[1].y }, { v3[0].x, v3[0].y, v3[1].x, v3[1].y } };
                u64 t[4];
                dyadic_redc<4, 2>(t, aa, bb, p, ninv);
#pragma unroll
                for (int j = 0; j < 4; j++)
                    x[batch * 4 + j] = t[j];
                __builtin_amdgcn_sched_barrier(0);
            }
        }

        template <int LOGN, int LZ, bool DY, bool WHOLE = false, bool QUARTER = false>
        __global__ __launch_bounds__(1 << (LOGN - 6), 4) void ntt_inv_half_kernel(u64 *__restrict__ data,
                                                                                  const PrimeDev *__restrict__ primes,
                                                                                  RowMap map, std::size_t nrows,
                                                                                  std::size_t chunk,
                                                                                  const u64 *__restrict__ src,
                                                                                  std::size_t src_poly_stride,
                                                                                  LiveSlots live, DyadicSrc dy,
                                                                                  int canonical = 0)
        {
            static_assert(!WHOLE || !DY, "whole-row form: plain transforms");
            static_assert(!QUARTER || (!DY && !WHOLE), "quarter-row form: plain transforms");
            constexpr int T = LOGN - 1;
            constexpr int LOGR = WHOLE ? T : (QUARTER ? T + 2 : LOGN);
            constexpr int N = 1 << LOGR;
            extern __shared__ u64 lds[];
            const int wave_base = __builtin_amdgcn_readfirstlane(static_cast<int>(threadIdx.x) & ~63);
            int half = 0, position;
            std::size_t poly;
            if constexpr (WHOLE)
            {
                const std::size_t slot = blockIdx.x >> 3, npolys = nrows / map.rows;
                const std::size_t v = static_cast<std::size_t>(blockIdx.x & 7u) * chunk + slot;
                if (slot >= chunk || v >= npolys * static_cast<std::size_t>(live.n))
                    return;
                poly = v % npolys;
                position = static_cast<int>(v / npolys);
            }
            else if constexpr (DY)
            {
                const unsigned xcd = blockIdx.x & 7u;
                const std::size_t slot = blockIdx.x >> 3, npolys = nrows / map.rows;
                half = static_cast<int>(slot & 1);
                const std::size_t v = static_cast<std::size_t>(xcd) * chunk + (slot >> 1);
                if ((slot >> 1) >= chunk || v >= npolys * static_cast<std::size_t>(live.n))
                    return;
                const int nr = live.n / 3;
                const std::size_t pr = v / 3;
                position = static_cast<int>(v - pr * 3) * nr + static_cast<int>(pr / npolys);
                poly = pr % npolys;
            }
            else if constexpr (QUARTER)
            {
                const std::size_t slot = blockIdx.x >> 3, npolys = nrows / map.rows;
                half = static_cast<int>(slot & 3);
                const std::size_t v = static_cast<std::size_t>(blockIdx.x & 7u) * chunk + (slot >> 2);
                if ((slot >> 2) >= chunk || v >= npolys * static_cast<std::size_t>(live.n))
                    return;
                poly = v % npolys;
                position = static_cast<int>(v / npolys);
            }
            else if (!half_block_map(blockIdx.x, nrows / map.rows, live.n, chunk, poly, position, half))
                return;
            const std::size_t row = poly * map.rows + live.slot[position];
            const unsigned short pid = map.prime[row % map.rows];
            const PrimeDev P = primes[pid];
            constexpr bool FP = LZ == 2;
            static_assert(!FP || !DY, "the floating-point instance serves plain half transforms only");
            const u64 p = P.p, two_p = FP ? fp_bits(P.p_d) : P.two_p;
            const u64 *tw = FP ? reinterpret_cast<const u64 *>(P.inv_d) : P.inv;
            const int gbase = half << T;
            u64 *halfp = data + (row << LOGR) + gbase;
            const u64 *inp = src ? src + (row / map.rows) * src_poly_stride + ((row % map.rows) << LOGR) + gbase : halfp;
            u64 x[32];
            const u64 neg_p = FP ? fp_bits(P.pinv_d) : 0 - p;
            const u64 rdp = LZ == 1 ? P.rdp : (LZ == 3 ? static_cast<u64>(__float_as_uint(small_quot_const(p))) : 0);
            {
                const int jloc = Arr<T, 4>::tid_index(fresh_tid(wave_base)), jl = Arr<T, 4>::tid_index(fresh_tid(wave_base));
                u64x2 tg0[FinalStage<T>::SG * FinalStage<T>::NTW];
                if constexpr (!DY)
                    FirstStage<T, 0, LZ>::load(tg0, tw, gbase + jloc, N);
                if constexpr (DY)
                {
                    const int slot = live.slot[position], I = slot / dy.kb, r = slot - I * dy.kb;
                    const u64 *xr = dy.x + poly * dy.item_stride + (static_cast<std::size_t>(r) << LOGN) + gbase;
                    const std::size_t ps = dy.poly_stride;
                    if (dy.square)
                    {
                        if (I == 1)
                            h_load_dyadic2<T, false, true>(x, xr, xr + ps, jl, p, P.ninv);
                        else
                            h_load_dyadic2<T, true>(x, xr + (I >> 1) * ps, nullptr, jl, p, P.ninv);
                    }
                    else if (I == 1)
                        h_load_dyadic4<T>(x, xr, xr + 3 * ps, xr + ps, xr + 2 * ps, jl, p, P.ninv);
                    else if (I == 0)
                        h_load_dyadic2<T>(x, xr, xr + 2 * ps, jl, p, P.ninv);
                    else
                        h_load_dyadic2<T>(x, xr + ps, xr + 3 * ps, jl, p, P.ninv);
                    FirstStage<T, 0, LZ>::load(tg0, tw, gbase + jloc, N);
                }
                else
                {
#pragma unroll
                    for (int s = 0; s < 32; s += 2)
                    {
                        const ulonglong2 v = *reinterpret_cast<const ulonglong2 *>(inp + jl + Arr<T, 4>::slot_index(s));
                        x[s] = FP ? fp_bits(fp_from_u64(v.x)) : v.x;
                        x[s + 1] = FP ? fp_bits(fp_from_u64(v.y)) : v.y;
                    }
                }
                __builtin_amdgcn_sched_barrier(0);
                ZeroPairs zp1;
                if constexpr (LZ == 1)
                    zp1.init();
                FirstPipe<T, 0, LZ, FinalStage<T>::PIPE && !(DY && kLazy<LZ>) && !(WHOLE && LZ == 0)>::run(x, tg0, tw, gbase + jloc, N, neg_p,
                                                                                                         two_p, rdp, zp1);
            }
            const int jb3 = gbase + Arr<T, 3>::tid_index(fresh_tid(wave_base));
            u64 w0[kIL], ws0[kIL];
            RoundStageInv<T, 3, false, 0, LZ>::load(w0, ws0, tw, jb3, N);
            __builtin_amdgcn_sched_barrier(0);
            h_exchange<T, 4, 3>(x, lds, fresh_tid(wave_base));
            ZeroPairs zp;
            if constexpr (kLazy<LZ>)
                zp.init();
            RoundPipeInv<T, 3, false, LZ>::run(x, w0, ws0, tw, jb3, N, two_p, neg_p, rdp, zp);
            const int jb2 = gbase + Arr<T, 2>::tid_index(fresh_tid(wave_base));
            RoundStageInv<T, 2, false, 0, LZ>::load(w0, ws0, tw, jb2, N);
            __builtin_amdgcn_sched_barrier(0);
            h_exchange<T, 3, 2>(x, lds, fresh_tid(wave_base));
            if constexpr (kLazy<LZ>)
                zp.init();
            RoundPipeInv<T, 2, false, LZ>::run(x, w0, ws0, tw, jb2, N, two_p, neg_p, rdp, zp);
            RoundStageInv<T, 1, true, 0, LZ>::load(w0, ws0, tw, gbase, N);
            h_exchange<T, 2, 1>(x, lds, fresh_tid(wave_base));
            if constexpr (kLazy<LZ>)
                zp.init();
            if constexpr (WHOLE)
            {
                RoundPipeInv<T, 1, true, LZ, 0, 3>::run(x, w0, ws0, tw, gbase, N, two_p, neg_p, rdp, zp);
                if constexpr (FP)
                {
                    const double pd = fp_of(two_p), pinv = fp_of(neg_p);
                    const double c_sum = static_cast<double>(P.inv_n), c_diff = static_cast<double>(P.inv_n_w);
#pragma unroll
                    for (int s2 = 0; s2 < 16; s2++)
                    {
                        const double u = fp_of(x[s2]), v = fp_of(x[s2 | 16]);
                        x[s2] = fp_bits(fp_mulmod(u + v, c_sum, pd, pinv));
                        x[s2 | 16] = fp_bits(fp_mulmod(u - v, c_diff, pd, pinv));
                    }
                }
                else
                {
                    const u64 addend = kLazy<LZ> ? (0 - neg_p) << InvLazy<T, LZ>::shift(T - 1) : two_p;
#pragma unroll
                    for (int s2 = 0; s2 < 16; s2++)
                    {
                        const u64 u = x[s2], v = x[s2 | 16];
                        u64 tt = u + v;
                        if (LZ == 0)
                            tt = tt >= two_p ? tt - two_p : tt;
                        u64 a0 = mulmod_lazy_hs<true>(tt, P.inv_n, P.inv_n_shoup, neg_p);
                        u64 a1 = mulmod_lazy_hs<true>(u - v + addend, P.inv_n_w, P.inv_n_w_shoup, neg_p);
                        if (canonical)
                        {
                            a0 = a0 >= p ? a0 - p : a0;
                            a1 = a1 >= p ? a1 - p : a1;
                        }
                        x[s2] = a0;
                        x[s2 | 16] = a1;
                    }
                }
            }
            else
                RoundPipeInv<T, 1, true, LZ>::run(x, w0, ws0, tw, gbase, N, two_p, neg_p, rdp, zp);
            {
                const int jb = Arr<T, 1>::tid_index(fresh_tid(wave_base));
#pragma unroll
                for (int s = 0; s < 32; s += 2)
                {
                    if constexpr (FP)
                        store_nt(halfp + jb + Arr<T, 1>::slot_index(s), fp_to_u64(fp_canonical(fp_of(x[s]), fp_of(two_p), fp_of(neg_p))),
                                 fp_to_u64(fp_canonical(fp_of(x[s + 1]), fp_of(two_p), fp_of(neg_p))));
                    else
                        store_nt(halfp + jb + Arr<T, 1>::slot_index(s), x[s], x[s + 1]);
                }
            }
        }

        __global__ __launch_bounds__(256) void ntt_inv_top_kernel(u64 *__restrict__ data,
                                                                  const PrimeDev *__restrict__ primes, RowMap map,
                                                                  int logn, std::size_t npairs, int flags)
        {
            const std::size_t stride = static_cast<std::size_t>(gridDim.x) * blockDim.x;
            const std::size_t half = static_cast<std::size_t>(1) << (logn - 1);
            for (std::size_t i = blockIdx.x * static_cast<std::size_t>(blockDim.x) + threadIdx.x; i < npairs; i += stride)
            {
                const std::size_t row = i >> (logn - 2);
                const std::size_t off = (i & ((half >> 1) - 1)) * 2;
                const unsigned short pid = map.prime[row % map.rows];
                if (pid == kSkipRow)
                    continue;
                const PrimeDev &P = primes[pid];
                const u64 p = P.p, two_p = P.two_p;
                u64 *lo = data + (row << logn) + off;
                u64 *hi = lo + half;
                const ulonglong2 a = *reinterpret_cast<const ulonglong2 *>(lo);
                const ulonglong2 b = *reinterpret_cast<const ulonglong2 *>(hi);
                ulonglong2 r0, r1;
                u64 t0 = a.x + b.x, t1 = a.y + b.y;
                t0 = t0 >= two_p ? t0 - two_p : t0;
                t1 = t1 >= two_p ? t1 - two_p : t1;
                r0.x = mulmod_lazy(t0, P.inv_n, P.inv_n_shoup, p);
                r0.y = mulmod_lazy(t1, P.inv_n, P.inv_n_shoup, p);
                r1.x = mulmod_lazy(a.x - b.x + two_p, P.inv_n_w, P.inv_n_w_shoup, p);
                r1.y = mulmod_lazy(a.y - b.y + two_p, P.inv_n_w, P.inv_n_w_shoup, p);
                if (flags & kNttCanonical)
                {
                    r0.x = r0.x >= p ? r0.x - p : r0.x;
                    r0.y = r0.y >= p ? r0.y - p : r0.y;
                    r1.x = r1.x >= p ? r1.x - p : r1.x;
                    r1.y = r1.y >= p ? r1.y - p : r1.y;
                }
                *reinterpret_cast<ulonglong2 *>(lo) = r0;
                *reinterpret_cast<ulonglong2 *>(hi) = r1;
            }
        }

        __global__ __launch_bounds__(256) void ntt_inv_top2_kernel(u64 *__restrict__ data, const PrimeDev *__restrict__ primes,
                                                                   RowMap map, int logn, std::size_t nitems, int flags)
        {
            const std::size_t stride = static_cast<std::size_t>(gridDim.x) * blockDim.x;
            const std::size_t quarter = static_cast<std::size_t>(1) << (logn - 2);
            for (std::size_t i = blockIdx.x * static_cast<std::size_t>(blockDim.x) + threadIdx.x; i < nitems; i += stride)
            {
                const std::size_t row = i >> (logn - 3);
                const std::size_t off = (i & ((quarter >> 1) - 1)) * 2;
                const unsigned short pid = map.prime[row % map.rows];
                if (pid == kSkipRow)
                    continue;
                const PrimeDev &P = primes[pid];
                const u64 p = P.p, two_p = P.two_p;
                const u64x2 WA = ((tw_global_t)P.inv)[2], WB = ((tw_global_t)P.inv)[3];
                u64 *q0 = data + (row << logn) + off;
                ulonglong2 x[4], y[4];
#pragma unroll
                for (int r = 0; r < 4; r++)
                    x[r] = *reinterpret_cast<const ulonglong2 *>(q0 + r * quarter);
                const auto lazy_pair = [&](u64 u, u64 v, u64 w, u64 ws, u64 &s, u64 &d) {
                    u64 tt = u + v;
                    s = tt >= two_p ? tt - two_p : tt;
                    d = mulmod_lazy(u - v + two_p, w, ws, p);
                };
                const auto last_pair = [&](u64 u, u64 v, u64 &lo, u64 &hi) {
                    u64 tt = u + v;
                    tt = tt >= two_p ? tt - two_p : tt;
                    lo = mulmod_lazy(tt, P.inv_n, P.inv_n_shoup, p);
                    hi = mulmod_lazy(u - v + two_p, P.inv_n_w, P.inv_n_w_shoup, p);
                    if (flags & kNttCanonical)
                    {
                        lo = lo >= p ? lo - p : lo;
                        hi = hi >= p ? hi - p : hi;
                    }
                };
                u64 s01, d01, s23, d23;
                lazy_pair(x[0].x, x[1].x, WA.x, WA.y, s01, d01);
                lazy_pair(x[2].x, x[3].x, WB.x, WB.y, s23, d23);
                last_pair(s01, s23, y[0].x, y[2].x);
                last_pair(d01, d23, y[1].x, y[3].x);
                lazy_pair(x[0].y, x[1].y, WA.x, WA.y, s01, d01);
                lazy_pair(x[2].y, x[3].y, WB.x, WB.y, s23, d23);
                last_pair(s01, s23, y[0].y, y[2].y);
                last_pair(d01, d23, y[1].y, y[3].y);
#pragma unroll
                for (int r = 0; r < 4; r++)
                    *reinterpret_cast<ulonglong2 *>(q0 + r * quarter) = y[r];
            }
        }

        template <int LOGN>
        hipError_t launch_half_inv(const Engine &e, u64 *data, std::size_t nrows, const RowMap &map, int flags,
                                   const u64 *src = nullptr, std::size_t src_poly_stride = 0,
                                   const DyadicSrc *dyadic = nullptr)
        {
            constexpr int T = LOGN - 1;
            if (fp64_enabled() && (flags & (kNttAnyRep | kNttCanonical)) != 0 && !dyadic)
            {
                RowMap a, b;
                if (split_by_fp(e, map, a, b))
                {
                    const hipError_t err = launch_half_inv<LOGN>(e, data, nrows, a, flags, src, src_poly_stride);
                    return err != hipSuccess ? err : launch_half_inv<LOGN>(e, data, nrows, b, flags, src, src_poly_stride);
                }
            }
            const std::size_t lds_bytes = static_cast<std::size_t>(hpad(1 << (T - 1))) * 8;
            if (nrows % map.rows != 0)
                return hipErrorInvalidValue;
            const LiveSlots live = live_slots(map);
            if (live.n == 0)
                return hipSuccess;
            const std::size_t chunk = ((nrows / map.rows) * live.n + 7) / 8;
            const std::size_t blocks = chunk * 16;
            if (blocks > 0x7fffffffull)
                return hipErrorInvalidValue;
            bool did_quarter = false;
            {
                ProfScope prof(e, "ntt_inv_half", transformed_rows(nrows, map));
                static const bool exact_only = std::getenv("SEALHIP_NTT_EXACT_INV") != nullptr;
                bool lazy = (flags & (kNttAnyRep | kNttCanonical)) != 0 && !exact_only;
                bool dense = lazy;
                for (int i = 0; dense && i < live.n; i++)
                    dense = bounds::inv_dense_admits(kInvLayers<LOGN>, e.tables[map.prime[live.slot[i]]].p);
                for (int i = 0; lazy && i < live.n; i++)
                    lazy = bounds::inv_lazy_admits(kInvLayers<LOGN>, e.tables[map.prime[live.slot[i]]].p);
                dense = dense && !lazy;
                bool fp = (flags & (kNttAnyRep | kNttCanonical)) != 0 && fp64_enabled() && !dyadic;
                for (int i = 0; fp && i < live.n; i++)
                    fp = e.tables[map.prime[live.slot[i]]].p < kFpPrimeBound;
                const DyadicSrc dy = dyadic ? *dyadic : DyadicSrc{};
                if constexpr (LOGN <= 15)
                {
                    if (!dyadic && !(flags & kNttDeferTop))
                    {
                        const std::size_t wlds = static_cast<std::size_t>(hpad(1 << (LOGN - 1))) * 8;
                        const int canon = (flags & kNttCanonical) ? 1 : 0;
#define SEALHIP_INV_WHOLE(LZ_)                                                                                          \
    ntt_inv_half_kernel<LOGN + 1, LZ_, false, true>                                                                      \
        <<<static_cast<unsigned>(chunk * 8), 1 << (LOGN - 5), wlds, e.lane().stream>>>(                                  \
            data, e.d_primes, map, nrows, chunk, src, src_poly_stride, live, dy, canon)
                        bool lazy_w = lazy, dense_w = (lazy || dense);
                        for (int i = 0; lazy_w && i < live.n; i++)
                            lazy_w = bounds::inv_lazy_admits(kInvLayers<LOGN + 1>, e.tables[map.prime[live.slot[i]]].p);
                        for (int i = 0; dense_w && i < live.n; i++)
                            dense_w = bounds::inv_dense_admits(kInvLayers<LOGN + 1>, e.tables[map.prime[live.slot[i]]].p);
                        if (fp)
                            SEALHIP_INV_WHOLE(2);
                        else if (lazy_w)
                            SEALHIP_INV_WHOLE(1);
                        else if (dense_w)
                            SEALHIP_INV_WHOLE(3);
                        else
                            SEALHIP_INV_WHOLE(0);
#undef SEALHIP_INV_WHOLE
                        return hipGetLastError();
                    }
                }
                if constexpr (LOGN == 16)
                {
                    if (!dyadic && !(flags & kNttDeferTop))
                    {
                        constexpr int QL = LOGN - 1;
                        const std::size_t qlds = static_cast<std::size_t>(hpad(1 << (QL - 2))) * 8;
                        const std::size_t qblocks = chunk * 32;
                        if (qblocks > 0x7fffffffull)
                            return hipErrorInvalidValue;
                        bool lazy_q = (flags & (kNttAnyRep | kNttCanonical)) != 0 && !exact_only, dense_q = lazy_q;
                        for (int i = 0; lazy_q && i < live.n; i++)
                            lazy_q = bounds::inv_lazy_admits(kInvLayers<QL>, e.tables[map.prime[live.slot[i]]].p);
                        for (int i = 0; dense_q && i < live.n; i++)
                            dense_q = bounds::inv_dense_admits(kInvLayers<QL>, e.tables[map.prime[live.slot[i]]].p);
#define SEALHIP_INV_QUARTER(LZ_)                                                                                          \
    ntt_inv_half_kernel<QL, LZ_, false, false, true>                                                                        \
        <<<static_cast<unsigned>(qblocks), 1 << (QL - 6), qlds, e.lane().stream>>>(data, e.d_primes, map, nrows, chunk, src, \
                                                                                    src_poly_stride, live, dy)
                        if (fp)
                            SEALHIP_INV_QUARTER(2);
                        else if (lazy_q)
                            SEALHIP_INV_QUARTER(1);
                        else if (dense_q)
                            SEALHIP_INV_QUARTER(3);
                        else
                            SEALHIP_INV_QUARTER(0);
#undef SEALHIP_INV_QUARTER
                        hipError_t qerr = hipGetLastError();
                        if (qerr != hipSuccess)
                            return qerr;
                        did_quarter = true;
                    }
                }
                if (!did_quarter)
                {
#define SEALHIP_INV_HALF(LZ_, DY_)                                                                                    \
    ntt_inv_half_kernel<LOGN, LZ_, DY_><<<static_cast<unsigned>(blocks), 1 << (LOGN - 6), lds_bytes, e.lane().stream>>>( \
        data, e.d_primes, map, nrows, chunk, src, src_poly_stride, live, dy)
                if (dyadic)
                {
                    if (lazy)
                        SEALHIP_INV_HALF(1, true);
                    else if (dense)
                        SEALHIP_INV_HALF(3, true);
                    else
                        SEALHIP_INV_HALF(0, true);
                }
                else if (fp)
                    SEALHIP_INV_HALF(2, false);
                else if (lazy)
                    SEALHIP_INV_HALF(1, false);
                else if (dense)
                    SEALHIP_INV_HALF(3, false);
                else
                    SEALHIP_INV_HALF(0, false);
#undef SEALHIP_INV_HALF
                hipError_t err = hipGetLastError();
                if (err != hipSuccess)
                    return err;
                }
            }
            if (did_quarter)
            {
                const std::size_t nitems = nrows << (LOGN - 3);
                std::size_t grid = (nitems + 255) / 256;
                if (grid > 256u * 32u)
                    grid = 256u * 32u;
                ProfScope prof(e, "ntt_inv_top", 0);
                ntt_inv_top2_kernel<<<static_cast<unsigned>(grid), 256, 0, e.lane().stream>>>(data, e.d_primes, map, LOGN, nitems, flags);
                return hipGetLastError();
            }
            if (flags & kNttDeferTop)
                return hipSuccess;
            const std::size_t npairs = nrows << (LOGN - 2);
            std::size_t grid = (npairs + 255) / 256;
            if (grid > 256u * 32u)
                grid = 256u * 32u;
            ProfScope prof(e, "ntt_inv_top", transformed_rows(nrows, map));
            ntt_inv_top_kernel<<<static_cast<unsigned>(grid), 256, 0, e.lane().stream>>>(data, e.d_primes, map, LOGN, npairs,
                                                                               flags);
            return hipGetLastError();
        }

        template <int LOGN>
        hipError_t init_half_inv()
        {
            const int lds_bytes = hpad(1 << (LOGN - 2)) * 8;
            hipError_t err = hipSuccess;
            const void *inv[7] = { reinterpret_cast<const void *>(&ntt_inv_half_kernel<LOGN, 2, false>),
                                   reinterpret_cast<const void *>(&ntt_inv_half_kernel<LOGN, 1, false>),
                                   reinterpret_cast<const void *>(&ntt_inv_half_kernel<LOGN, 0, false>),
                                   reinterpret_cast<const void *>(&ntt_inv_half_kernel<LOGN, 3, false>),
                                   reinterpret_cast<const void *>(&ntt_inv_half_kernel<LOGN, 1, true>),
                                   reinterpret_cast<const void *>(&ntt_inv_half_kernel<LOGN, 3, true>),
                                   reinterpret_cast<const void *>(&ntt_inv_half_kernel<LOGN, 0, true>) };
            for (const void *f : inv)
            {
                err = hipFuncSetAttribute(f, hipFuncAttributeMaxDynamicSharedMemorySize, lds_bytes);
                if (err != hipSuccess)
                    return err;
            }
            if constexpr (LOGN == 15)
            {
                const void *quarter[4] = { reinterpret_cast<const void *>(&ntt_inv_half_kernel<LOGN, 2, false, false, true>),
                                           reinterpret_cast<const void *>(&ntt_inv_half_kernel<LOGN, 1, false, false, true>),
                                           reinterpret_cast<const void *>(&ntt_inv_half_kernel<LOGN, 3, false, false, true>),
                                           reinterpret_cast<const void *>(&ntt_inv_half_kernel<LOGN, 0, false, false, true>) };
                for (const void *f : quarter)
                {
                    err = hipFuncSetAttribute(f, hipFuncAttributeMaxDynamicSharedMemorySize, lds_bytes);
                    if (err != hipSuccess)
                        return err;
                }
            }
            if constexpr (LOGN <= 15)
            {
                const void *whole[4] = { reinterpret_cast<const void *>(&ntt_inv_half_kernel<LOGN + 1, 2, false, true>),
                                         reinterpret_cast<const void *>(&ntt_inv_half_kernel<LOGN + 1, 1, false, true>),
                                         reinterpret_cast<const void *>(&ntt_inv_half_kernel<LOGN + 1, 3, false, true>),
                                         reinterpret_cast<const void *>(&ntt_inv_half_kernel<LOGN + 1, 0, false, true>) };
                for (const void *f : whole)
                {
                    err = hipFuncSetAttribute(f, hipFuncAttributeMaxDynamicSharedMemorySize, hpad(1 << (LOGN - 1)) * 8);
                    if (err != hipSuccess)
                        return err;
                }
            }
            return err;
        }
    }

    hipError_t ntt_inv_half(const Engine &e, u64 *data, std::size_t nrows, const RowMap &map, int flags, const u64 *src,
                            std::size_t src_poly_stride)
    {
        switch (e.logn)
        {
        case 14: return launch_half_inv<14>(e, data, nrows, map, flags, src, src_poly_stride);
        case 15: return launch_half_inv<15>(e, data, nrows, map, flags, src, src_poly_stride);
        case 16: return launch_half_inv<16>(e, data, nrows, map, flags, src, src_poly_stride);
        default: return hipErrorInvalidValue;
        }
    }

    hipError_t ntt_inv_tensor(const Engine &e, u64 *data, std::size_t nrows, const RowMap &map, int flags, const u64 *x,
                              std::size_t item_stride, std::size_t poly_stride, int kb, bool square)
    {
        const DyadicSrc dy{ x, item_stride, poly_stride, kb, square ? 1 : 0 };
        switch (e.logn)
        {
        case 14: return launch_half_inv<14>(e, data, nrows, map, flags, nullptr, 0, &dy);
        case 15: return launch_half_inv<15>(e, data, nrows, map, flags, nullptr, 0, &dy);
        case 16: return launch_half_inv<16>(e, data, nrows, map, flags, nullptr, 0, &dy);
        default: return hipErrorInvalidValue;
        }
    }

    hipError_t ntt_inv_half_init()
    {
        hipError_t err = init_half_inv<14>();
        if (err == hipSuccess)
            err = init_half_inv<15>();
        if (err == hipSuccess)
            err = init_half_inv<16>();
        return err;
    }
}
```

gemini-seal_amd/csrc/pipeline.cpp:

```cpp
#include "engine.hpp"

#include <cmath>

#include <algorithm>
#include <cstdlib>
#include <vector>

namespace sealhip
{
    namespace
    {
        std::size_t workspace_budget_bytes(const Engine &e)
        {
            Lane &l = e.lane();
            if (l.ws_budget)
                return l.ws_budget;
            static const std::size_t env_budget = [] {
                if (const char *env = std::getenv("SEALHIP_WORKSPACE_MB"))
                {
                    std::size_t mb = static_cast<std::size_t>(std::strtoull(env, nullptr, 10));
                    return (mb < 64 ? std::size_t(64) : mb) << 20;
                }
                return std::size_t(0);
            }();
// ... 61 lines not shown
                m.prime[j * rows + r] = (only < 0 || only == j) ? static_cast<unsigned short>(r) : kSkipRow;
        return m;
    }

    static std::size_t switch_key_item_bytes(Engine &e, int k)
    {
        LevelTools &lt = e.level(k);
        const std::size_t N = e.n;
        const std::size_t rows = static_cast<std::size_t>(k + e.nsp), nd = static_cast<std::size_t>(lt.h_ks.nd);
        const bool ckks = e.scheme == 2;
        const bool strict_bfv = e.mode_strict && !ckks;
        const std::size_t w_coeff = (ckks || strict_bfv) ? static_cast<std::size_t>(k) * N : 0;
        return (w_coeff + nd * rows * N + 2 * rows * N + 2 * static_cast<std::size_t>(k) * N) * sizeof(u64);
    }

    namespace
    {
        unsigned *sink_at(Engine &e, std::size_t off)
        {
            Lane &l = e.lane();
            return l.tsink_cur ? l.tsink_cur + l.tsink_base + off : nullptr;
        }
        struct SinkArm
        {
            Lane &l;
            SinkArm(Engine &e, unsigned *flags) : l(e.lane())
            {
                l.tsink_arm = flags;
            }
            ~SinkArm()
            {
                l.tsink_arm = nullptr;
            }
        };
        struct FloorRestore
        {
            Lane &l;
            std::size_t floor;
            explicit FloorRestore(Engine &e) : l(e.lane()), floor(l.ws_floor)
            {}
            ~FloorRestore()
            {
                l.ws_floor = floor;
            }
        };
    }

    namespace
    {
        struct KsRows
        {
            const u64 *inb;
            std::size_t inb_stride;
        };
        KsRows ks_digits(Engine &e, LevelTools &lt, int k, const u64 *tg, std::size_t target_stride, std::size_t m, u64 *coeff,
                         u64 *ext, int dj0, int dj1)
        {
            const KsDev &h = lt.h_ks;
            const std::size_t N = e.n;
            const int rows = k + e.nsp;
            const bool ckks = e.scheme == 2;
            const bool strict_bfv = e.mode_strict && !ckks;
            const RowMap map_q = lt.map_q;
            const RowMap map_rows = lt.map_key;
            const std::size_t ext_item = static_cast<std::size_t>(rows) * N;
            const std::size_t ext_digit = ext_item * m;
            const u64 *src = tg;
            std::size_t src_stride = target_stride;
            if (ckks)
            {
                if (ntt_can_gather(e))
                    check(launch_intt_from(e, coeff, tg, target_stride, m * k, map_q, kNttCanonical | kNttAnyRep),
                          "intt(target)");
                else
                {
                    check(launch_copy_rows(e, tg, target_stride, coeff, static_cast<std::size_t>(k) * N, m, k), "copy");
                    check(launch_ntt(e, coeff, m * k, map_q, true, kNttCanonical), "intt(target)");
                }
                src = coeff;
                src_stride = static_cast<std::size_t>(k) * N;
            }
            const bool gather = e.nsp == 1 && ntt_can_gather(e);
            bool need_any = false, need_barrett = false;
            for (int a = 0; a < k; a++)
                for (int b = 0; b < rows; b++)
                {
                    const u64 ps = e.key_moduli[h.row_prime[a]], pd = e.key_moduli[h.row_prime[b]];
                    need_any = need_any || (a != b && ps > pd);
                    need_barrett = need_barrett || (a != b && ps >= 2 * pd);
                }
            int modup_mode = need_barrett ? 1 : (need_any ? 2 : 0);
            if (modup_mode == 2)
            {
                u64 pmax = 0;
                for (int r = 0; r < rows; r++)
                    pmax = std::max(pmax, e.key_moduli[h.row_prime[r]]);
                if (bounds::fwd_lazy_admits(pmax, e.logn))
                    modup_mode = 0;
            }
            if (!gather)
                check(launch_ks_modup(e, lt.d_ks, h, src, src_stride, ext, ext_item, ext_digit, m, -1), "modup");
            for (int j = dj0; j < dj1; j++)
            {
                RowMap mj = map_rows;
                const int r0 = j * e.nsp, r1 = std::min(r0 + e.nsp, k);
                for (int r = r0; r < r1; r++)
                    mj.prime[r] = kSkipRow;
                if (gather)
                {
                    NttSource ns{};
                    ns.base[0] = src;
                    ns.poly_stride[0] = src_stride;
                    ns.reduce_mode = modup_mode;
                    const u64 p_src = e.key_moduli[h.row_prime[j]];
                    for (int r = 0; r < rows; r++)
                    {
                        if (r == j)
                        {
                            ns.code[r] = kSkipRow;
                            continue;
                        }
                        const u64 p_dst = e.key_moduli[h.row_prime[r]];
                        ns.code[r] = static_cast<unsigned short>(j | (p_src <= p_dst ? 0 : kSrcReduce));
                    }
                    check(launch_ntt_gather(e, ext + j * ext_digit, m * rows, mj, ns, kNttAnyRep | kNttApprox), "ntt(ext, gathered)");
                }
                else
                    check(launch_ntt(e, ext + j * ext_digit, m * rows, mj, false, kNttAnyRep), "ntt(ext)");
            }
            const u64 *inb = tg;
            std::size_t inb_stride = target_stride;
            if (strict_bfv)
            {
                if (ntt_can_gather(e))
                {
                    NttSource ns{};
                    ns.base[0] = tg;
                    ns.poly_stride[0] = target_stride;
                    for (int r = 0; r < k; r++)
                        ns.code[r] = static_cast<unsigned short>(r);
                    check(launch_ntt_gather(e, coeff, m * k, map_q, ns, kNttAnyRep | kNttApprox), "ntt(target, gathered)");
                }
                else
                {
                    check(launch_copy_rows(e, tg, target_stride, coeff, static_cast<std::size_t>(k) * N, m, k), "copy");
                    check(launch_ntt(e, coeff, m * k, map_q, false, 0), "ntt(target)");
                }
                inb = coeff;
                inb_stride = static_cast<std::size_t>(k) * N;
            }
            return KsRows{ inb, inb_stride };
        }

        void ks_finish(Engine &e, LevelTools &lt, int k, u64 *prod, u64 *temp, u64 *ctp, std::size_t ct_stride, const u64 *c0p,
                       std::size_t c0_stride, std::size_t m, unsigned *sink, bool one_component = false)
        {
            const KsDev &h = lt.h_ks;
            const std::size_t N = e.n;
            const int rows = k + e.nsp;
            const bool ckks = e.scheme == 2;
            const RowMap map_q = lt.map_q;
            const std::size_t ext_item = static_cast<std::size_t>(rows) * N;
            RowMap map_rows = lt.map_key;
            u64 *const prod_rows = one_component ? prod - ext_item : prod;
            const std::size_t npolys = one_component ? m : 2 * m, prod_stride = one_component ? 2 * ext_item : ext_item;
            const int lead = one_component ? rows : 0;
            if (one_component)
            {
                if (c0p || sink || ct_stride != 2 * static_cast<std::size_t>(k) * N || 2 * rows > kMaxRows)
                    throw std::logic_error("internal: one-component mod-down misused");
                map_rows.rows = 2 * rows;
                for (int r = 0; r < rows; r++)
                {
                    map_rows.prime[rows + r] = map_rows.prime[r];
                    map_rows.prime[r] = kSkipRow;
                }
            }
            if (!ckks)
            {
                const bool defer = ntt_can_defer_top(e, k);
                check(launch_ntt(e, prod_rows, m * 2 * rows, map_rows, true, (defer ? kNttDeferTop : 0) | kNttAnyRep), "intt(prod)");
                SinkArm arm(e, sink);
                check(launch_ks_moddown_bfv(e, lt.d_ks, h, prod, prod_stride, ctp, ct_stride, npolys, defer, c0p, c0_stride),
                      "moddown_bfv");
                return;
            }
            const u64 p_special = (ckks && e.nsp == 1) ? e.key_moduli[h.row_prime[k]] : 0;
            bool fold_ok = ckks && e.nsp == 1 && ntt_can_gather(e);
            for (int r = 0; fold_ok && r < k; r++)
            {
                const u64 q = e.key_moduli[h.row_prime[r]];
                fold_ok = p_special <= q || (p_special < 2 * q && bounds::fwd_lazy_admits(q, e.logn));
            }
            const bool fold_pre = fold_ok;
            const bool fold_top = fold_pre && ntt_can_defer_top(e, k);
            const bool fold_store = fold_top && ntt_can_fuse_moddown(e, k, p_special);
            check(launch_ntt(e, prod_rows, m * 2 * rows, skip_map(map_rows, lead + k, lead + rows), true,
                             kNttAnyRep | (fold_top ? kNttDeferTop : 0)),
                  "intt(special)");
            if (fold_pre)
            {
                NttSource ns{};
                ns.base[0] = prod;
                ns.poly_stride[0] = prod_stride;
                ns.reduce_mode = fold_store ? 7 : (fold_top ? 5 : 4);
                if (fold_store)
                {
                    ns.md.inv_p = lt.d_ks->invP;
                    ns.md.inv_p_shoup = lt.d_ks->invP_shoup;
                    ns.md.prod = prod;
                    ns.md.prod_stride = prod_stride;
                    ns.md.ct = ctp;
                    ns.md.ct_stride = ct_stride;
                    ns.md.c0_src = c0p;
                    ns.md.c0_stride = c0_stride;
                    ns.md.tflags = sink;
                }
                ns.aux_p = p_special;
                ns.aux_cr1 = HostModulus(p_special).cr1;
                {
                    const HostNttTables &tb = e.tables[h.row_prime[k]];
                    ns.aux_top[0] = tb.inv_n;
                    ns.aux_top[1] = tb.inv_n_shoup;
                    ns.aux_top[2] = tb.inv_n_w;
                    ns.aux_top[3] = tb.inv_n_w_shoup;
                }
                for (int r = 0; r < k; r++)
                    ns.code[r] = static_cast<unsigned short>(k);
                check(launch_ntt_gather(e, temp, npolys * k, map_q, ns, kNttAnyRep), "ntt(temp, gathered from the special row)");
            }
            else
            {
                check(launch_ks_moddown_pre(e, lt.d_ks, h, prod, prod_stride, temp, static_cast<std::size_t>(k) * N, npolys),
                      "moddown_pre");
                if (ckks)
                    check(launch_ntt(e, temp, npolys * k, map_q, false, kNttAnyRep), "ntt(temp)");
                else
                    check(launch_ntt(e, prod_rows, m * 2 * rows, skip_map(map_rows, lead, lead + k), true, kNttAnyRep), "intt(prod)");
            }
            if (!fold_store)
            {
                SinkArm arm(e, sink);
                check(launch_ks_moddown_post(e, lt.d_ks, h, prod, prod_stride, temp, static_cast<std::size_t>(k) * N, ctp,
                                             ct_stride, npolys, 1, c0p, c0_stride),
                      "moddown_post");
            }
        }

        void ks_finish_rescale(Engine &e, LevelTools &lt, int k, const u64 *base, std::size_t base_stride, u64 *acc, u64 *temp,
                               u64 *out, std::size_t m, unsigned *sink)
        {
            if (e.scheme != 2 || k < 2 || !lt.d_ksr)
                throw std::logic_error("internal: merged rescale misused");
            const KsRescaleDev &h = lt.h_ksr;
            const std::size_t N = e.n;
            const int rows = k + e.nsp;
            const std::size_t ext_item = static_cast<std::size_t>(rows) * N;
            check(launch_ks_rescale_fold(e, lt.d_ksr, h, base, base_stride, acc, ext_item, 2 * m), "rescale_fold");
            check(launch_ntt(e, acc, m * 2 * rows, skip_map(lt.map_key, k - 1, rows), true, kNttCanonical), "intt(dropped)");
            check(launch_ks_moddown_rescale_pre(e, lt.d_ksr, h, acc, ext_item, temp, 2 * m), "moddown_rescale_pre");
            check(launch_ntt(e, temp, m * 2 * (k - 1), e.level_host(k - 1).map_q, false, kNttCanonical | kNttStrict), "ntt(temp)");
            SinkArm arm(e, sink);
            check(launch_ks_moddown_rescale_post(e, lt.d_ksr, h, base, base_stride, acc, ext_item, temp, out, 2 * m),
                  "moddown_rescale_post");
        }
    }

    void op_switch_key(Engine &e, int k, u64 *ct, std::size_t ct_stride, const u64 *target, std::size_t target_stride,
                       std::size_t count, const KSwitchKey &key, const u64 *c0_src, std::size_t c0_stride, const KsSplit *split)
    {
        if (k > e.k_first)
            throw std::invalid_argument("key switching needs a ciphertext level");
        LevelTools &lt = e.level(k);
        const KsDev &h = lt.h_ks;
        const bool finish = split && split->partial_sum;
        const bool partial = split && split->partial_out;
        if (!finish && static_cast<int>(key.n_digits) < h.nd)
            throw std::invalid_argument("kswitch_keys is not valid for encryption parameters");
        const int dj0 = partial ? split->j0 : 0, dj1 = partial ? split->j1 : h.nd;
        if (dj0 < 0 || dj0 > dj1 || dj1 > h.nd)
            throw std::invalid_argument("digit range out of bounds");
        const std::size_t N = e.n;
        const int rows = k + e.nsp, nd = h.nd;
        const bool ckks = e.scheme == 2;
        const bool strict_bfv = e.mode_strict && !ckks;
        const std::size_t w_coeff = (ckks || strict_bfv) ? static_cast<std::size_t>(k) * N : 0;
        const std::size_t w_ext = static_cast<std::size_t>(nd) * rows * N;
        const std::size_t w_prod = 2ull * rows * N;
        const std::size_t w_temp = 2ull * k * N;
        const std::size_t per_item = switch_key_item_bytes(e, k);
        if (per_item != (w_coeff + w_ext + w_prod + w_temp) * sizeof(u64))
            throw std::logic_error("internal: arena accounting mismatch");
        const RowMap map_rows = lt.map_key;
        for_chunks(e, count, per_item, 4, [&](std::size_t off, std::size_t m) {
            u64 *coeff = w_coeff ? e.ws_alloc(w_coeff * m) : nullptr;
            u64 *ext = e.ws_alloc(w_ext * m);
            u64 *prod = e.ws_alloc(w_prod * m);
            u64 *temp = e.ws_alloc(w_temp * m);
            if (partial)
                prod = split->partial_out + off * w_prod;
            if (finish)
                prod = split->partial_sum + off * w_prod;
            const u64 *tg = finish ? nullptr : target + off * target_stride;
            u64 *ctp = partial ? nullptr : ct + off * ct_stride;
            const u64 *c0p = c0_src ? c0_src + off * c0_stride : nullptr;
            const std::size_t ext_item = static_cast<std::size_t>(rows) * N;
            const std::size_t ext_digit = ext_item * m;

            if (finish)
                check(launch_poly_op(e, PolyOp::Mod63, prod, nullptr, 0, prod, m * 2 * rows, map_rows), "mod(partial sum)");
            if (!finish)
            {
                const KsRows in_bundle = ks_digits(e, lt, k, tg, target_stride, m, coeff, ext, dj0, dj1);
                check(launch_ks_mac(e, lt.d_ks, h, in_bundle.inb, in_bundle.inb_stride, ext, ext_item, ext_digit, key.d_data, prod,
                                    w_prod, m, dj0, dj1),
                      "mac");
            }
            if (partial)
                return;
            ks_finish(e, lt, k, prod, temp, ctp, ct_stride, c0p, c0_stride, m, sink_at(e, off));
        });
    }

    static std::size_t switch_key_rescale_item_bytes(Engine &e, int k)
    {
        const std::size_t N = e.n, rows = static_cast<std::size_t>(k + e.nsp);
        const std::size_t nd = static_cast<std::size_t>(e.level(k).h_ks.nd);
        return (static_cast<std::size_t>(k) * N + nd * rows * N + 2 * rows * N + 2 * static_cast<std::size_t>(k - 1) * N) *
               sizeof(u64);
    }

    void op_switch_key_rescale(Engine &e, int k, const u64 *base, std::size_t base_stride, const u64 *target,
                               std::size_t target_stride, std::size_t count, const KSwitchKey &key, u64 *out)
    {
        if (e.scheme != 2)
            throw std::invalid_argument("the merged rescale is a CKKS operation");
        if (k > e.k_first)
            throw std::invalid_argument("key switching needs a ciphertext level");
        if (k < 2)
            throw std::invalid_argument("end of modulus switching chain reached");
        LevelTools &lt = e.level_rescale(k);
        const KsDev &h = lt.h_ks;
        if (static_cast<int>(key.n_digits) < h.nd)
            throw std::invalid_argument("kswitch_keys is not valid for encryption parameters");
        const std::size_t N = e.n;
        const int rows = k + e.nsp, nd = h.nd;
        const std::size_t w_coeff = static_cast<std::size_t>(k) * N;
        const std::size_t w_ext = static_cast<std::size_t>(nd) * rows * N;
        const std::size_t w_prod = 2ull * rows * N;
        const std::size_t w_temp = 2ull * (k - 1) * N;
        const std::size_t per_item = switch_key_rescale_item_bytes(e, k);
        if (per_item != (w_coeff + w_ext + w_prod + w_temp) * sizeof(u64))
            throw std::logic_error("internal: arena accounting mismatch");
        for_chunks(e, count, per_item, 4, [&](std::size_t off, std::size_t m) {
            u64 *coeff = e.ws_alloc(w_coeff * m);
            u64 *ext = e.ws_alloc(w_ext * m);
            u64 *prod = e.ws_alloc(w_prod * m);
            u64 *temp = e.ws_alloc(w_temp * m);
            const std::size_t ext_item = static_cast<std::size_t>(rows) * N;
            const KsRows in_bundle = ks_digits(e, lt, k, target + off * target_stride, target_stride, m, coeff, ext, 0, nd);
            check(launch_ks_mac(e, lt.d_ks, h, in_bundle.inb, in_bundle.inb_stride, ext, ext_item, ext_item * m, key.d_data, prod,
                                w_prod, m, 0, nd),
                  "mac");
            ks_finish_rescale(e, lt, k, base + off * base_stride, base_stride, prod, temp, out + off * w_temp, m, sink_at(e, off));
        });
    }

    void op_modup(Engine &e, int k, int bundle, u64 *ext, std::size_t count)
    {
        LevelTools &lt = e.level(k);
        if (k > e.k_first || bundle < 0 || bundle >= lt.h_ks.nd)
            throw std::invalid_argument("modup_rns: src_bundle_index out of bound");
        const std::size_t stride = static_cast<std::size_t>(k + e.nsp) * e.n;
        check(launch_ks_modup(e, lt.d_ks, lt.h_ks, ext, stride, ext, stride, 0, count, bundle), "modup");
    }

    void op_rescale_special_inplace(Engine &e, int k, u64 *poly, std::size_t count)
    {
        if (k > e.k_first)
            throw std::invalid_argument("rescale_special needs a ciphertext level");
        LevelTools &lt = e.level(k);
        const std::size_t N = e.n;
        const int rows = k + e.nsp;
        const std::size_t per_item = static_cast<std::size_t>(k) * N * sizeof(u64);
        for_chunks(e, count, per_item, 1, [&](std::size_t off, std::size_t m) {
            u64 *temp = e.ws_alloc(static_cast<std::size_t>(k) * N * m);
            u64 *p = poly + off * rows * N;
            check(launch_ks_moddown_pre(e, lt.d_ks, lt.h_ks, p, static_cast<std::size_t>(rows) * N, temp,
                                        static_cast<std::size_t>(k) * N, m),
                  "moddown_pre");
            if (e.scheme == 2)
                check(launch_ntt(e, temp, m * k, lt.map_q, false, 0), "ntt(temp)");
            else
                check(launch_ntt(e, p, m * rows, skip_map(lt.map_key, 0, k), true, 0), "intt(poly)");
            check(launch_ks_moddown_post(e, lt.d_ks, lt.h_ks, p, static_cast<std::size_t>(rows) * N, temp,
                                         static_cast<std::size_t>(k) * N, nullptr, 0, m, 0),
                  "moddown_post");
        });
    }

    BfvMulPlan plan_bfv_multiply(Engine &e, int k, int sa, int sb, bool square)
    {
        if (e.scheme != 1)
            throw std::invalid_argument("plan_bfv_multiply: BFV contexts only");
        if (sa < 2 || sb < 2 || (square && (sa != 2 || sb != 2)))
            throw std::invalid_argument("plan_bfv_multiply: operand sizes (the square path takes size-2 operands)");
        LevelTools &lt = e.level_host(k);
        const HostRnsTool &hr = *lt.host_rns;
        BfvMulPlan p{};
        p.k = k;
        p.B = static_cast<int>(hr.B_size);
        p.nB = static_cast<int>(hr.Bsk.size());
        p.square = square;
        u64 max_q = 0, max_b = 0;
        for (int i = 0; i < k; i++)
            max_q = std::max(max_q, hr.q[i]);
        for (int j = 0; j < p.nB; j++)
            max_b = std::max(max_b, hr.Bsk[j]);
        p.redc_small = bounds::behz_redc_small(k, p.B, max_q, max_b);
        const int kb = k + p.nB, sin = square ? sa : sa + sb, dest = sa + sb - 1;
        p.gather = ntt_can_gather(e) && sin * kb <= kMaxRows;
        p.defer = ntt_can_defer_top(e, k);
        p.fused_tensor = p.gather && p.defer && sa == 2 && sb == 2 && dest * kb <= kMaxRows;
        p.tensor_apx = true;
        for (int r = 0; r < k; r++)
        {
            p.fused_tensor = p.fused_tensor && bounds::tensor_admits_4p(e.key_moduli[r]);
            p.tensor_apx = p.tensor_apx && bounds::tensor_admits_apx(e.key_moduli[r]);
        }
        for (int j = 0; j < p.nB; j++)
            p.fused_tensor = p.fused_tensor && bounds::tensor_admits_2p(e.tables[lt.map_qbsk.prime[k + j]].p);
        p.lift_top = p.fused_tensor && bfv_lift_can_apply_top(e, k, p.redc_small);
        if (p.lift_top && e.mode_strict)
        {
            RowMap bsk{};
            bsk.rows = p.nB;
            for (int j = 0; j < p.nB; j++)
                bsk.prime[j] = lt.map_qbsk.prime[k + j];
            p.lift_top = ntt_strict_top_done_ok(e, bsk);
        }
        const int code = k > 32 ? kBehzStepwise : p.redc_small && k <= bounds::kBehzExactMaxK ? k : kBehzGeneric;
        p.lift_kernel = p.floor_kernel = code;
        p.deferred_top = p.fused_tensor ? 2 : p.defer ? 1 : 0;
        return p;
    }

    void op_bfv_multiply(Engine &e, int k, const u64 *a, int sa, const u64 *b, int sb, std::size_t count, u64 *out)
    {
        LevelTools &lt = e.level(k);
        const RnsDev &h = lt.h_rns;
        const std::size_t N = e.n;
        const bool sq = b == nullptr;
        if (sq && (sa != 2 || sb != 2))
            throw std::logic_error("op_bfv_multiply: the square path takes size-2 operands");
        const BfvMulPlan plan = plan_bfv_multiply(e, k, sa, sb, sq);
        if (plan.nB != h.nB || plan.redc_small != (h.redc_small != 0))
            throw std::logic_error("op_bfv_multiply: the plan and the level's device constants disagree");
        const bool gather = plan.gather, defer = plan.defer, fused_tensor = plan.fused_tensor, tensor_apx = plan.tensor_apx,
                   lift_top = plan.lift_top;
        const int nB = h.nB, kb = k + nB, sin = sq ? sa : sa + sb, dest = sa + sb - 1;
        const std::size_t w_x = static_cast<std::size_t>(sin) * kb * N;
        const std::size_t w_d = static_cast<std::size_t>(dest) * kb * N;
        const std::size_t poly_q = static_cast<std::size_t>(k) * N, poly_x = static_cast<std::size_t>(kb) * N;
        for_chunks(e, count, (w_x + w_d) * sizeof(u64), 2, [&](std::size_t off, std::size_t m) {
            u64 *X = e.ws_alloc(w_x * m);
            u64 *D = e.ws_alloc(w_d * m);
// ... 1397 lines not shown
```

Before: 23980.

## Fuse key-switch inner product into inverse NTT load for BFV

Adds an inverse-NTT kernel variant that computes the key-switch multiply-accumulate (digits times key) on load, using Montgomery reduction, instead of writing the product to memory in a separate MAC kernel. Moddown then applies inverse-N constants pre-scaled by 2^64 mod p to undo the Montgomery factor. This removes one full pass of writes and reads of the product buffer. The fused path is limited to one special prime, log n below 16, at most seven digits and primes that satisfy new accumulation bounds, and it adds kernel register pressure.

Measured after the change: 23580. -1.7%, worse.

```diff
diff --git a/gemini-seal_amd/csrc/devmath.hpp b/gemini-seal_amd/csrc/devmath.hpp
--- a/gemini-seal_amd/csrc/devmath.hpp
+++ b/gemini-seal_amd/csrc/devmath.hpp
@@ -24,6 +24,7 @@
         const double *fwd_d;
         const double *inv_d;
         double p_d, pinv_d;
+        u64 inv_n_m, inv_n_m_shoup, inv_n_w_m, inv_n_w_m_shoup;
     };
 
     constexpr double kTwo52 = 4503599627370496.0;
diff --git a/gemini-seal_amd/csrc/engine.cpp b/gemini-seal_amd/csrc/engine.cpp
--- a/gemini-seal_amd/csrc/engine.cpp
+++ b/gemini-seal_amd/csrc/engine.cpp
@@ -108,6 +108,13 @@
             d.inv_n_w = tb.inv_n_w;
             d.inv_n_w_shoup = tb.inv_n_w_shoup;
             {
+                const u64 r64 = static_cast<u64>((static_cast<u128>(1) << 64) % tb.p);
+                d.inv_n_m = mulmod(tb.inv_n, r64, tb.p);
+                d.inv_n_m_shoup = shoup(d.inv_n_m, tb.p);
+                d.inv_n_w_m = mulmod(tb.inv_n_w, r64, tb.p);
+                d.inv_n_w_m_shoup = shoup(d.inv_n_w_m, tb.p);
+            }
+            {
                 u64 inv = tb.p;
                 for (int it = 0; it < 6; it++)
                     inv *= 2 - tb.p * inv;
diff --git a/gemini-seal_amd/csrc/engine.hpp b/gemini-seal_amd/csrc/engine.hpp
--- a/gemini-seal_amd/csrc/engine.hpp
+++ b/gemini-seal_amd/csrc/engine.hpp
@@ -451,6 +451,10 @@
                                 const RowMap &map, int flags);
     hipError_t launch_intt_tensor(const Engine &e, u64 *data, const u64 *x, std::size_t item_stride, std::size_t poly_stride,
                                   int kb, std::size_t nrows, const RowMap &map, int flags, bool square = false);
+    bool ks_mac_can_fuse(const Engine &e, int k);
+    hipError_t launch_intt_ks_mac(const Engine &e, const KsDev &h, u64 *prod, std::size_t count, const RowMap &map_key,
+                                  const u64 *inb, std::size_t inb_stride, const u64 *ext, std::size_t ext_stride,
+                                  std::size_t ext_digit_stride, const u64 *key);
     hipError_t launch_divround_bfv(const Engine &e, const RnsDev *d, const RnsDev &h, const u64 *in,
                                    std::size_t in_stride, u64 *out, std::size_t out_stride, std::size_t count,
                                    int out_rows);
@@ -493,7 +497,8 @@
                                      std::size_t prod_stride, u64 *temp, std::size_t temp_stride, std::size_t npolys);
     hipError_t launch_ks_moddown_bfv(const Engine &e, const KsDev *d, const KsDev &h, const u64 *prod,
                                      std::size_t prod_stride, u64 *ct, std::size_t ct_item_stride, std::size_t npolys,
-                                     bool top_deferred, const u64 *c0_src = nullptr, std::size_t c0_stride = 0);
+                                     bool top_deferred, const u64 *c0_src = nullptr, std::size_t c0_stride = 0,
+                                     bool montgomery = false);
     hipError_t launch_ks_moddown_post(const Engine &e, const KsDev *d, const KsDev &h, u64 *prod,
                                       std::size_t prod_stride, const u64 *temp, std::size_t temp_stride, u64 *ct,
                                       std::size_t ct_item_stride, std::size_t npolys, int add_into_ct,
diff --git a/gemini-seal_amd/csrc/keyswitch.hip b/gemini-seal_amd/csrc/keyswitch.hip
--- a/gemini-seal_amd/csrc/keyswitch.hip
+++ b/gemini-seal_amd/csrc/keyswitch.hip
@@ -276,7 +276,7 @@
 
         template <bool DEFER>
         __device__ __forceinline__ void row_pair(const u64 *__restrict__ row, std::size_t c_lo, std::size_t half,
-                                                 const PrimeDev &P, u64 &x_lo, u64 &x_hi)
+                                                 const PrimeDev &P, u64 &x_lo, u64 &x_hi, int mont = 0)
         {
             const u64 u = row[c_lo], v = row[c_lo + half];
             if (!DEFER)
@@ -287,8 +287,8 @@
             }
             u64 tt = u + v;
             tt = tt >= P.two_p ? tt - P.two_p : tt;
-            x_lo = mulmod_lazy(tt, P.inv_n, P.inv_n_shoup, P.p);
-            x_hi = mulmod_lazy(u - v + P.two_p, P.inv_n_w, P.inv_n_w_shoup, P.p);
+            x_lo = mulmod_lazy(tt, mont ? P.inv_n_m : P.inv_n, mont ? P.inv_n_m_shoup : P.inv_n_shoup, P.p);
+            x_hi = mulmod_lazy(u - v + P.two_p, mont ? P.inv_n_w_m : P.inv_n_w, mont ? P.inv_n_w_m_shoup : P.inv_n_w_shoup, P.p);
         }
 
         template <bool DEFER, bool ONE>
@@ -298,7 +298,8 @@
                                                                           std::size_t prod_stride, u64 *__restrict__ ct,
                                                                           std::size_t ct_item_stride, std::size_t npolys,
                                                                           int logn, const u64 *__restrict__ c0_src,
-                                                                          std::size_t c0_stride, unsigned *__restrict__ tflags)
+                                                                          std::size_t c0_stride, unsigned *__restrict__ tflags,
+                                                                          int mont)
         {
             const std::size_t N = static_cast<std::size_t>(1) << logn, half = N >> 1;
             const int k = d->k, nsp = d->nsp;
@@ -313,7 +314,7 @@
             {
                 const PrimeDev &S = primes[d->row_prime[k]];
                 u64 sv[2];
-                row_pair<DEFER>(pp + static_cast<std::size_t>(k) * N, c, half, S, sv[0], sv[1]);
+                row_pair<DEFER>(pp + static_cast<std::size_t>(k) * N, c, half, S, sv[0], sv[1], mont);
 #pragma unroll
                 for (int h = 0; h < 2; h++)
                     sred[h] = neg_mod(barrett_reduce_63(sv[h], S.p, S.cr1), S.p);
@@ -336,7 +337,7 @@
                     {
                         const PrimeDev &S = primes[d->row_prime[k + j]];
                         u64 sv[2];
-                        row_pair<DEFER>(pp + static_cast<std::size_t>(k + j) * N, c, half, S, sv[0], sv[1]);
+                        row_pair<DEFER>(pp + static_cast<std::size_t>(k + j) * N, c, half, S, sv[0], sv[1], mont);
 #pragma unroll
                         for (int h = 0; h < 2; h++)
                         {
@@ -348,7 +349,7 @@
                     temp[1] = barrett_reduce_128(lo[1], hi[1], Q.p, Q.cr0, Q.cr1);
                 }
                 u64 pv[2];
-                row_pair<DEFER>(pp + static_cast<std::size_t>(q) * N, c, half, Q, pv[0], pv[1]);
+                row_pair<DEFER>(pp + static_cast<std::size_t>(q) * N, c, half, Q, pv[0], pv[1], mont);
                 u64 *pc = ct + (poly >> 1) * ct_item_stride + ((poly & 1) * static_cast<std::size_t>(k) + q) * N + c;
 #pragma unroll
                 for (int h = 0; h < 2; h++)
@@ -573,15 +574,18 @@
 
     hipError_t launch_ks_moddown_bfv(const Engine &e, const KsDev *d, const KsDev &h, const u64 *prod,
                                      std::size_t prod_stride, u64 *ct, std::size_t ct_item_stride, std::size_t npolys,
-                                     bool top_deferred, const u64 *c0_src, std::size_t c0_stride)
+                                     bool top_deferred, const u64 *c0_src, std::size_t c0_stride, bool montgomery)
     {
         if (!npolys)
             return hipSuccess;
+        if (montgomery && !top_deferred)
+            return hipErrorInvalidValue;
         const std::size_t lanes = npolys << (e.logn - 1);
         ProfScope prof(e, "ks_moddown_bfv", 0);
 #define SEALHIP_MODDOWN_BFV(DEFER_, ONE_)                                                                            \
     ks_moddown_bfv_kernel<DEFER_, ONE_><<<blocks_for(lanes), kThreads, 0, e.lane().stream>>>(                              \
-        d, e.d_primes, prod, prod_stride, ct, ct_item_stride, npolys, e.logn, c0_src, c0_stride, e.lane().tsink_arm)
+        d, e.d_primes, prod, prod_stride, ct, ct_item_stride, npolys, e.logn, c0_src, c0_stride, e.lane().tsink_arm,          \
+        montgomery ? 1 : 0)
         if (top_deferred && h.nsp == 1)
             SEALHIP_MODDOWN_BFV(true, true);
         else if (top_deferred)
diff --git a/gemini-seal_amd/csrc/ntt.hip b/gemini-seal_amd/csrc/ntt.hip
--- a/gemini-seal_amd/csrc/ntt.hip
+++ b/gemini-seal_amd/csrc/ntt.hip
@@ -554,6 +554,37 @@
         return ntt_inv_tensor(e, data, nrows, map, flags, x, item_stride, poly_stride, kb, square);
     }
 
+    bool ks_mac_can_fuse(const Engine &e, int k)
+    {
+        if (e.scheme != 1 || e.nsp != 1 || !ntt_can_gather(e) || !ntt_can_defer_top(e, k) || k < 1 || k > e.k_first)
+            return false;
+        if (e.logn == 16)
+            return false;
+        const int nd = k;
+        for (int r = 0; r <= k; r++)
+        {
+            const u64 p = e.key_moduli[r < k ? r : e.k_first];
+            if (!bounds::ks_fused_admits(p, e.logn, nd) || (fp64_enabled() && p < kFpPrimeBound))
+                return false;
+        }
+        return true;
+    }
+
+    hipError_t launch_intt_ks_mac(const Engine &e, const KsDev &h, u64 *prod, std::size_t count, const RowMap &map_key,
+                                  const u64 *inb, std::size_t inb_stride, const u64 *ext, std::size_t ext_stride,
+                                  std::size_t ext_digit_stride, const u64 *key)
+    {
+        if (!ks_mac_can_fuse(e, h.k) || h.nsp != 1 || h.nd != h.k)
+            return hipErrorInvalidValue;
+        if (count == 0)
+            return hipSuccess;
+        int flags = kNttDeferTop | kNttAnyRep;
+        if (e.mode_strict)
+            flags |= kNttStrict;
+        return ntt_inv_ks_mac(e, prod, count * 2 * static_cast<std::size_t>(h.k + 1), map_key, flags, ext, ext_stride, ext_digit_stride,
+                              inb, inb_stride, key, static_cast<std::size_t>(h.n_total) << e.logn, h.nd, h.k);
+    }
+
     hipError_t launch_ntt(const Engine &e, u64 *data, size_t nrows, const RowMap &map, bool inverse, int flags)
     {
         if (nrows == 0)
diff --git a/gemini-seal_amd/csrc/ntt_bounds.hpp b/gemini-seal_amd/csrc/ntt_bounds.hpp
--- a/gemini-seal_amd/csrc/ntt_bounds.hpp
+++ b/gemini-seal_amd/csrc/ntt_bounds.hpp
@@ -380,5 +380,51 @@
         }
         static_assert(ks_rescale_sum_fits(64, kDotAccOperandBits) && !ks_rescale_sum_fits(65, kDotAccOperandBits),
                       "the last prime and up to 63 special primes of 61 bits: 64 dropped primes fit, 65 would not");
+
+        constexpr int ks_fused_digit_mult(int logn)
+        {
+            return fwd_apx_output_mult(logn, true);
+        }
+        constexpr u128 ks_fused_sum_max(u64 p, int logn, int nd)
+        {
+            const u128 d = static_cast<u128>(ks_fused_digit_mult(logn)) * p - 1, max = ~static_cast<u128>(0);
+            if (d > max / (p - 1))
+                return max;
+            const u128 one = d * (p - 1);
+            return one > max / static_cast<u128>(nd) ? max : one * static_cast<u128>(nd);
+        }
+        constexpr u128 ks_fused_mid_max(u64 p, int logn, int nd)
+        {
+            const u128 d = static_cast<u128>(ks_fused_digit_mult(logn)) * p - 1, half = (static_cast<u128>(1) << 32) - 1;
+            return static_cast<u128>(nd) * (half * ((p - 1) >> 32) + (d >> 32) * half);
+        }
+        constexpr u128 ks_fused_high_max(u64 p, int logn, int nd)
+        {
+            const u128 d = static_cast<u128>(ks_fused_digit_mult(logn)) * p - 1;
+            return static_cast<u128>(nd) * ((d >> 32) * ((p - 1) >> 32)) + static_cast<u128>(nd - 1);
+        }
+        constexpr bool ks_fused_sum_ok(u64 p, int logn, int nd)
+        {
+            return nd >= 1 && p >= 2 && logn >= kMinHalfLogn && logn <= kMaxHalfLogn &&
+                   static_cast<u128>(ks_fused_digit_mult(logn)) * p <= kWord && ks_fused_mid_max(p, logn, nd) < kWord &&
+                   ks_fused_high_max(p, logn, nd) < kWord && ks_fused_sum_max(p, logn, nd) <= static_cast<u128>(p) * kWord;
+        }
+        constexpr int ks_fused_prime_bits(int logn, int nd)
+        {
+            int bits = 0;
+            for (int b = 2; b <= kMaxPrimeBits; b++)
+                if (ks_fused_sum_ok(max_prime_of_bits(b), logn, nd))
+                    bits = b;
+            return bits;
+        }
+        constexpr int kKsFusedMaxDigits = 7;
+        constexpr bool ks_fused_admits(u64 p, int logn, int nd)
+        {
+            return nd >= 1 && nd <= kKsFusedMaxDigits && logn >= kMinHalfLogn && logn <= kMaxHalfLogn && p <= max_prime_of_bits(ks_fused_prime_bits(logn, nd));
+        }
+        static_assert(ks_fused_prime_bits(15, 7) == 55 && ks_fused_prime_bits(14, 7) == 55 && ks_fused_prime_bits(16, 7) == 55,
+                      "seven digits (the headline configuration): primes below 2^55, 7 * 62 p^2 <= p 2^64 at log n = 15");
+        static_assert(ks_fused_prime_bits(14, 1) == 58 && ks_fused_prime_bits(14, 3) == 56,
+                      "one digit: 58p below 2^64 for primes below 2^58; three digits at log n = 14: below 2^56");
     }
 }
diff --git a/gemini-seal_amd/csrc/ntt_half.hpp b/gemini-seal_amd/csrc/ntt_half.hpp
--- a/gemini-seal_amd/csrc/ntt_half.hpp
+++ b/gemini-seal_amd/csrc/ntt_half.hpp
@@ -15,6 +15,9 @@
     SEALHIP_INTERNAL hipError_t ntt_inv_tensor(const Engine &e, u64 *data, std::size_t nrows, const RowMap &map, int flags,
                                                const u64 *x, std::size_t item_stride, std::size_t poly_stride, int kb,
                                                bool square);
+    SEALHIP_INTERNAL hipError_t ntt_inv_ks_mac(const Engine &e, u64 *prod, std::size_t nrows, const RowMap &map, int flags,
+                                               const u64 *ext, std::size_t ext_item, std::size_t ext_digit, const u64 *inb,
+                                               std::size_t inb_stride, const u64 *key, std::size_t key_comp, int nd, int k);
     SEALHIP_INTERNAL hipError_t ntt_fwd_half_init();
     SEALHIP_INTERNAL hipError_t ntt_inv_half_init();
 
diff --git a/gemini-seal_amd/csrc/ntt_inv.hip b/gemini-seal_amd/csrc/ntt_inv.hip
--- a/gemini-seal_amd/csrc/ntt_inv.hip
+++ b/gemini-seal_amd/csrc/ntt_inv.hip
@@ -234,6 +234,33 @@
             int kb;
             int square;
         };
+        template <int IL>
+        __device__ __forceinline__ void redc_lockstep(u64 (&t)[IL], const u64 (&lo)[IL], const u64 (&hi)[IL], u64 (&cy)[IL], u64 p,
+                                                      u64 ninv)
+        {
+            u64 m[IL], A[IL], B[IL], carry[IL], mh[IL];
+            u32 cb[IL];
+            const u32 p0 = static_cast<u32>(p), p1 = static_cast<u32>(p >> 32);
+#pragma unroll
+            for (int j = 0; j < IL; j++)
+                m[j] = lo[j] * ninv;
+#pragma unroll
+            for (int j = 0; j < IL; j++)
+                A[j] = mad64v<true>(static_cast<u32>(m[j] >> 32), p0, static_cast<u64>(__umulhi(static_cast<u32>(m[j]), p0)), cy[j]);
+#pragma unroll
+            for (int j = 0; j < IL; j++)
+                asm volatile("v_mad_u64_u32 %0, %1, %2, %3, %4" : "=v"(B[j]), "=s"(carry[j]) : "v"(static_cast<u32>(m[j])), "s"(p1), "v"(A[j]));
+#pragma unroll
+            for (int j = 0; j < IL; j++)
+                asm volatile("v_cndmask_b32_e64 %0, 0, 1, %1" : "=v"(cb[j]) : "s"(carry[j]));
+#pragma unroll
+            for (int j = 0; j < IL; j++)
+                mh[j] = mad64v<true>(static_cast<u32>(m[j] >> 32), p1,
+                                     static_cast<u64>(static_cast<u32>(B[j] >> 32)) | (static_cast<u64>(cb[j]) << 32), cy[j]);
+#pragma unroll
+            for (int j = 0; j < IL; j++)
+                t[j] = hi[j] + mh[j] + (lo[j] != 0);
+        }
         template <int IL, int NP>
         __device__ __forceinline__ void dyadic_redc(u64 (&t)[IL], const u64 (&a)[NP][IL], const u64 (&b)[NP][IL], u64 p, u64 ninv)
         {
@@ -258,9 +285,7 @@
                     H[j] = q == 0 ? mul64v<false>(static_cast<u32>(a[q][j] >> 32), static_cast<u32>(b[q][j] >> 32), cy[j])
                                   : mad64v<false>(static_cast<u32>(a[q][j] >> 32), static_cast<u32>(b[q][j] >> 32), H[j], cy[j]);
             }
-            u64 lo[IL], hi[IL], m[IL], A[IL], B[IL], carry[IL], mh[IL];
-            u32 cb[IL];
-            const u32 p0 = static_cast<u32>(p), p1 = static_cast<u32>(p >> 32);
+            u64 lo[IL], hi[IL];
 #pragma unroll
             for (int j = 0; j < IL; j++)
             {
@@ -270,24 +295,8 @@
                     X += P0[q][j];
                 lo[j] = static_cast<u64>(X);
                 hi[j] = static_cast<u64>(X >> 64);
-                m[j] = lo[j] * ninv;
-            }
-#pragma unroll
-            for (int j = 0; j < IL; j++)
-                A[j] = mad64v<true>(static_cast<u32>(m[j] >> 32), p0, static_cast<u64>(__umulhi(static_cast<u32>(m[j]), p0)), cy[j]);
-#pragma unroll
-            for (int j = 0; j < IL; j++)
-                asm volatile("v_mad_u64_u32 %0, %1, %2, %3, %4" : "=v"(B[j]), "=s"(carry[j]) : "v"(static_cast<u32>(m[j])), "s"(p1), "v"(A[j]));
-#pragma unroll
-            for (int j = 0; j < IL; j++)
-                asm volatile("v_cndmask_b32_e64 %0, 0, 1, %1" : "=v"(cb[j]) : "s"(carry[j]));
-#pragma unroll
-            for (int j = 0; j < IL; j++)
-                mh[j] = mad64v<true>(static_cast<u32>(m[j] >> 32), p1,
-                                     static_cast<u64>(static_cast<u32>(B[j] >> 32)) | (static_cast<u64>(cb[j]) << 32), cy[j]);
-#pragma unroll
-            for (int j = 0; j < IL; j++)
-                t[j] = hi[j] + mh[j] + (lo[j] != 0);
+            }
+            redc_lockstep<IL>(t, lo, hi, cy, p, ninv);
         }
 
         template <int T, bool SAME = false, bool TWICE = false>
@@ -358,7 +367,136 @@
             }
         }
 
-        template <int LOGN, int LZ, bool DY, bool WHOLE = false, bool QUARTER = false>
+        struct KsMacSrc
+        {
+            const u64 *ext;
+            std::size_t ext_item, ext_digit;
+            const u64 *inb;
+            std::size_t inb_stride;
+            const u64 *key;
+            std::size_t key_comp;
+            int nd, k;
+        };
+        template <int IL, int NP, bool FIRST>
+        __device__ __forceinline__ void ksmac_acc(u64 (&L)[IL], u64 (&M)[IL], u64 (&H)[IL], u32 (&NC)[IL], u64 (&cy)[3][IL],
+                                                  const u64 (&a)[NP][IL], const u64 (&b)[NP][IL])
+        {
+#pragma unroll
+            for (int q = 0; q < NP; q++)
+            {
+                const bool first = FIRST && q == 0;
+                u64 cl[IL];
+#pragma unroll
+                for (int j = 0; j < IL; j++)
+                {
+                    if (first)
+                        L[j] = mul64v<false>(static_cast<u32>(a[q][j]), static_cast<u32>(b[q][j]), cy[2][j]);
+                    else
+                    {
+                        u64 d;
+                        asm volatile("v_mad_u64_u32 %0, %1, %2, %3, %4"
+                                     : "=v"(d), "=s"(cl[j])
+                                     : "v"(static_cast<u32>(a[q][j])), "v"(static_cast<u32>(b[q][j])), "v"(L[j]));
+                        L[j] = d;
+                    }
+                }
+#pragma unroll
+                for (int j = 0; j < IL; j++)
+                    M[j] = first ? mul64v<false>(static_cast<u32>(a[q][j]), static_cast<u32>(b[q][j] >> 32), cy[0][j])
+                                 : mad64v<false>(static_cast<u32>(a[q][j]), static_cast<u32>(b[q][j] >> 32), M[j], cy[0][j]);
+#pragma unroll
+                for (int j = 0; j < IL; j++)
+                    M[j] = mad64v<false>(static_cast<u32>(a[q][j] >> 32), static_cast<u32>(b[q][j]), M[j], cy[1][j]);
+#pragma unroll
+                for (int j = 0; j < IL; j++)
+                    H[j] = first ? mul64v<false>(static_cast<u32>(a[q][j] >> 32), static_cast<u32>(b[q][j] >> 32), cy[2][j])
+                                 : mad64v<false>(static_cast<u32>(a[q][j] >> 32), static_cast<u32>(b[q][j] >> 32), H[j], cy[2][j]);
+#pragma unroll
+                for (int j = 0; j < IL; j++)
+                {
+                    if (first)
+                        NC[j] = 0;
+                    else
+                        asm volatile("v_addc_co_u32_e64 %0, %1, %0, 0, %1" : "+v"(NC[j]), "+s"(cl[j]));
+                }
+            }
+        }
+        __host__ __device__ constexpr int ks_load_part(int s, int nd)
+        {
+            const int fit = (128 - 22 - 2 * s) / 8;
+            return fit < 1 ? 1 : (fit < nd ? fit : nd);
+        }
+        template <int ND, int J0, int J1, bool FIRST>
+        __device__ __forceinline__ void ksmac_part(u64 (&L)[2], u64 (&M)[2], u64 (&H)[2], u32 (&NC)[2], u64 (&cy)[3][2],
+                                                   const char *const (&dbase)[ND], const char *const (&kbase)[ND], unsigned off)
+        {
+            constexpr int NP = J1 - J0;
+            ulonglong2 vd[NP], vk[NP];
+#pragma unroll
+            for (int q = 0; q < NP; q++)
+            {
+                vd[q] = *reinterpret_cast<const ulonglong2 *>(dbase[J0 + q] + off);
+                vk[q] = *reinterpret_cast<const ulonglong2 *>(kbase[J0 + q] + off);
+            }
+            u64 a[NP][2], b[NP][2];
+#pragma unroll
+            for (int q = 0; q < NP; q++)
+            {
+                a[q][0] = vd[q].x;
+                a[q][1] = vd[q].y;
+                b[q][0] = vk[q].x;
+                b[q][1] = vk[q].y;
+            }
+            ksmac_acc<2, NP, FIRST>(L, M, H, NC, cy, a, b);
+        }
+        template <int T, int ND, int S = 0>
+        __device__ __forceinline__ void ksmac_batches(u64 (&x)[32], const char *const (&dbase)[ND], const char *const (&kbase)[ND],
+                                                      unsigned lane_off, u64 p, u64 ninv)
+        {
+            typedef unsigned __int128 u128;
+            constexpr int PART = ks_load_part(S, ND);
+            constexpr unsigned off_s = static_cast<unsigned>(Arr<T, 4>::slot_index(S)) * 8u;
+            const unsigned off = lane_off + off_s;
+            u64 L[2], M[2], H[2], cy[3][2] = {};
+            u32 NC[2];
+            ksmac_part<ND, 0, PART, true>(L, M, H, NC, cy, dbase, kbase, off);
+            if constexpr (PART < ND)
+            {
+                __builtin_amdgcn_sched_barrier(0);
+                ksmac_part<ND, PART, ND, false>(L, M, H, NC, cy, dbase, kbase, off);
+            }
+            u64 lo[2], hi[2], t[2];
+#pragma unroll
+            for (int j = 0; j < 2; j++)
+            {
+                const u128 X = (static_cast<u128>(H[j] + NC[j]) << 64) + (static_cast<u128>(M[j]) << 32) + L[j];
+                lo[j] = static_cast<u64>(X);
+                hi[j] = static_cast<u64>(X >> 64);
+            }
+            redc_lockstep<2>(t, lo, hi, cy[0], p, ninv);
+            x[S] = t[0];
+            x[S + 1] = t[1];
+            __builtin_amdgcn_sched_barrier(0);
+            if constexpr (S + 2 < 32)
+                ksmac_batches<T, ND, S + 2>(x, dbase, kbase, lane_off, p, ninv);
+        }
+        template <int T, int ND>
+        __device__ __forceinline__ void h_load_ksmac(u64 (&x)[32], const u64 *__restrict__ drow, std::size_t ext_digit,
+                                                     const u64 *__restrict__ own, int own_digit, const u64 *__restrict__ krow,
+                                                     std::size_t key_comp, int jloc, u64 p, u64 ninv)
+        {
+            static_assert(2 * ks_load_part(30, ND) >= ND, "at most two parts per batch");
+            const char *dbase[ND], *kbase[ND];
+#pragma unroll
+            for (int j = 0; j < ND; j++)
+            {
+                dbase[j] = reinterpret_cast<const char *>(j == own_digit ? own : drow + static_cast<std::size_t>(j) * ext_digit);
+                kbase[j] = reinterpret_cast<const char *>(krow + 2 * static_cast<std::size_t>(j) * key_comp);
+            }
+            ksmac_batches<T, ND>(x, dbase, kbase, static_cast<unsigned>(jloc) * 8u, p, ninv);
+        }
+
+        template <int LOGN, int LZ, bool DY, bool WHOLE = false, bool QUARTER = false, bool KS = false>
         __global__ __launch_bounds__(1 << (LOGN - 6), 4) void ntt_inv_half_kernel(u64 *__restrict__ data,
                                                                                   const PrimeDev *__restrict__ primes,
                                                                                   RowMap map, std::size_t nrows,
@@ -366,9 +504,10 @@
                                                                                   const u64 *__restrict__ src,
                                                                                   std::size_t src_poly_stride,
                                                                                   LiveSlots live, DyadicSrc dy,
-                                                                                  int canonical = 0)
+                                                                                  int canonical = 0, KsMacSrc ks = KsMacSrc{})
         {
             static_assert(!WHOLE || !DY, "whole-row form: plain transforms");
+            static_assert(!KS || (!DY && !WHOLE && !QUARTER && LZ != 2), "key-switch form: integer half-row instances");
             static_assert(!QUARTER || (!DY && !WHOLE), "quarter-row form: plain transforms");
             constexpr int T = LOGN - 1;
             constexpr int LOGR = WHOLE ? T : (QUARTER ? T + 2 : LOGN);
@@ -398,6 +537,17 @@
                 const std::size_t pr = v / 3;
                 position = static_cast<int>(v - pr * 3) * nr + static_cast<int>(pr / npolys);
                 poly = pr % npolys;
+            }
+            else if constexpr (KS)
+            {
+                const std::size_t slot = blockIdx.x >> 3, npolys = nrows / map.rows;
+                const std::size_t v = static_cast<std::size_t>(blockIdx.x & 7u) * chunk + slot;
+                if (slot >= chunk || v >= npolys * static_cast<std::size_t>(live.n) * 2)
+                    return;
+                const std::size_t ph = v / npolys;
+                poly = v - ph * npolys;
+                half = static_cast<int>(ph & 1);
+                position = static_cast<int>(ph >> 1);
             }
             else if constexpr (QUARTER)
             {
@@ -425,11 +575,40 @@
             const u64 neg_p = FP ? fp_bits(P.pinv_d) : 0 - p;
             const u64 rdp = LZ == 1 ? P.rdp : (LZ == 3 ? static_cast<u64>(__float_as_uint(small_quot_const(p))) : 0);
             {
-                const int jloc = Arr<T, 4>::tid_index(fresh_tid(wave_base)), jl = Arr<T, 4>::tid_index(fresh_tid(wave_base));
+                int jloc = Arr<T, 4>::tid_index(fresh_tid(wave_base));
+                const int jl = Arr<T, 4>::tid_index(fresh_tid(wave_base));
                 u64x2 tg0[FinalStage<T>::SG * FinalStage<T>::NTW];
-                if constexpr (!DY)
+                if constexpr (!DY && !KS)
                     FirstStage<T, 0, LZ>::load(tg0, tw, gbase + jloc, N);
-                if constexpr (DY)
+                if constexpr (KS)
+                {
+                    const int r = live.slot[position];
+                    const std::size_t item = poly >> 1, l = poly & 1;
+                    const std::size_t roff = (static_cast<std::size_t>(r) << LOGN) + gbase;
+                    const u64 *drow = ks.ext + item * ks.ext_item + roff, *own = ks.inb + item * ks.inb_stride + roff;
+                    const u64 *krow = ks.key + l * ks.key_comp + (static_cast<std::size_t>(pid) << LOGN) + gbase;
+                    const int own_digit = r < ks.k ? r : -1;
+#define SEALHIP_KS_LOAD(ND_)                                                                                          \
+    case ND_:                                                                                                         \
+        h_load_ksmac<T, ND_>(x, drow, ks.ext_digit, own, own_digit, krow, ks.key_comp, jl, p, P.ninv);               \
+        break;
+                    switch (ks.nd)
+                    {
+                        SEALHIP_KS_LOAD(1)
+                        SEALHIP_KS_LOAD(2)
+                        SEALHIP_KS_LOAD(3)
+                        SEALHIP_KS_LOAD(4)
+                        SEALHIP_KS_LOAD(5)
+                        SEALHIP_KS_LOAD(6)
+                    default:
+                        h_load_ksmac<T, bounds::kKsFusedMaxDigits>(x, drow, ks.ext_digit, own, own_digit, krow, ks.key_comp, jl, p,
+                                                                   P.ninv);
+                    }
+#undef SEALHIP_KS_LOAD
+                    jloc = Arr<T, 4>::tid_index(fresh_tid(wave_base));
+                    FirstStage<T, 0, LZ>::load(tg0, tw, gbase + jloc, N);
+                }
+                else if constexpr (DY)
                 {
                     const int slot = live.slot[position], I = slot / dy.kb, r = slot - I * dy.kb;
                     const u64 *xr = dy.x + poly * dy.item_stride + (static_cast<std::size_t>(r) << LOGN) + gbase;
@@ -463,7 +642,7 @@
                 ZeroPairs zp1;
                 if constexpr (LZ == 1)
                     zp1.init();
-                FirstPipe<T, 0, LZ, FinalStage<T>::PIPE && !(DY && kLazy<LZ>) && !(WHOLE && LZ == 0)>::run(x, tg0, tw, gbase + jloc, N, neg_p,
+                FirstPipe<T, 0, LZ, FinalStage<T>::PIPE && !((DY || KS) && kLazy<LZ>) && !(WHOLE && LZ == 0)>::run(x, tg0, tw, gbase + jloc, N, neg_p,
                                                                                                          two_p, rdp, zp1);
             }
             const int jb3 = gbase + Arr<T, 3>::tid_index(fresh_tid(wave_base));
@@ -632,10 +811,12 @@
         template <int LOGN>
         hipError_t launch_half_inv(const Engine &e, u64 *data, std::size_t nrows, const RowMap &map, int flags,
                                    const u64 *src = nullptr, std::size_t src_poly_stride = 0,
-                                   const DyadicSrc *dyadic = nullptr)
+                                   const DyadicSrc *dyadic = nullptr, const KsMacSrc *ksmac = nullptr)
         {
             constexpr int T = LOGN - 1;
-            if (fp64_enabled() && (flags & (kNttAnyRep | kNttCanonical)) != 0 && !dyadic)
+            if (ksmac && (dyadic || src || !(flags & kNttDeferTop) || !(flags & kNttAnyRep)))
+                return hipErrorInvalidValue;
+            if (fp64_enabled() && (flags & (kNttAnyRep | kNttCanonical)) != 0 && !dyadic && !ksmac)
             {
                 RowMap a, b;
                 if (split_by_fp(e, map, a, b))
@@ -665,10 +846,35 @@
                 for (int i = 0; lazy && i < live.n; i++)
                     lazy = bounds::inv_lazy_admits(kInvLayers<LOGN>, e.tables[map.prime[live.slot[i]]].p);
                 dense = dense && !lazy;
-                bool fp = (flags & (kNttAnyRep | kNttCanonical)) != 0 && fp64_enabled() && !dyadic;
+                bool fp = (flags & (kNttAnyRep | kNttCanonical)) != 0 && fp64_enabled() && !dyadic && !ksmac;
                 for (int i = 0; fp && i < live.n; i++)
                     fp = e.tables[map.prime[live.slot[i]]].p < kFpPrimeBound;
                 const DyadicSrc dy = dyadic ? *dyadic : DyadicSrc{};
+                if constexpr (LOGN == 16)
+                {
+                    if (ksmac)
+                        return hipErrorInvalidValue;
+                }
+                else if (ksmac)
+                {
+                    const std::size_t units = (nrows / map.rows) * static_cast<std::size_t>(live.n) * 2;
+                    std::size_t kchunk = (units + 7) / 8;
+                    kchunk += kchunk & 1;
+                    if (kchunk * 8 > 0x7fffffffull)
+                        return hipErrorInvalidValue;
+#define SEALHIP_INV_KS(LZ_)                                                                                            \
+    ntt_inv_half_kernel<LOGN, LZ_, false, false, false, true>                                                            \
+        <<<static_cast<unsigned>(kchunk * 8), 1 << (LOGN - 6), lds_bytes, e.lane().stream>>>(                            \
+            data, e.d_primes, map, nrows, kchunk, nullptr, 0, live, dy, 0, *ksmac)
+                    if (lazy)
+                        SEALHIP_INV_KS(1);
+                    else if (dense)
+                        SEALHIP_INV_KS(3);
+                    else
+                        SEALHIP_INV_KS(0);
+#undef SEALHIP_INV_KS
+                    return hipGetLastError();
+                }
                 if constexpr (LOGN <= 15)
                 {
                     if (!dyadic && !(flags & kNttDeferTop))
@@ -784,7 +990,7 @@
         {
             const int lds_bytes = hpad(1 << (LOGN - 2)) * 8;
             hipError_t err = hipSuccess;
-            const void *inv[7] = { reinterpret_cast<const void *>(&ntt_inv_half_kernel<LOGN, 2, false>),
+            const void *inv[7] = {                                    reinterpret_cast<const void *>(&ntt_inv_half_kernel<LOGN, 2, false>),
                                    reinterpret_cast<const void *>(&ntt_inv_half_kernel<LOGN, 1, false>),
                                    reinterpret_cast<const void *>(&ntt_inv_half_kernel<LOGN, 0, false>),
                                    reinterpret_cast<const void *>(&ntt_inv_half_kernel<LOGN, 3, false>),
@@ -797,6 +1003,18 @@
                 if (err != hipSuccess)
                     return err;
             }
+            if constexpr (LOGN <= 15)
+            {
+                const void *ksm[3] = { reinterpret_cast<const void *>(&ntt_inv_half_kernel<LOGN, 1, false, false, false, true>),
+                                       reinterpret_cast<const void *>(&ntt_inv_half_kernel<LOGN, 3, false, false, false, true>),
+                                       reinterpret_cast<const void *>(&ntt_inv_half_kernel<LOGN, 0, false, false, false, true>) };
+                for (const void *f : ksm)
+                {
+                    err = hipFuncSetAttribute(f, hipFuncAttributeMaxDynamicSharedMemorySize, lds_bytes);
+                    if (err != hipSuccess)
+                        return err;
+                }
+            }
             if constexpr (LOGN == 15)
             {
                 const void *quarter[4] = { reinterpret_cast<const void *>(&ntt_inv_half_kernel<LOGN, 2, false, false, true>),
@@ -848,6 +1066,25 @@
         case 14: return launch_half_inv<14>(e, data, nrows, map, flags, nullptr, 0, &dy);
         case 15: return launch_half_inv<15>(e, data, nrows, map, flags, nullptr, 0, &dy);
         case 16: return launch_half_inv<16>(e, data, nrows, map, flags, nullptr, 0, &dy);
+        default: return hipErrorInvalidValue;
+        }
+    }
+
+    hipError_t ntt_inv_ks_mac(const Engine &e, u64 *prod, std::size_t nrows, const RowMap &map, int flags, const u64 *ext,
+                              std::size_t ext_item, std::size_t ext_digit, const u64 *inb, std::size_t inb_stride, const u64 *key,
+                              std::size_t key_comp, int nd, int k)
+    {
+        if (map.rows != k + 1 || nd < 1 || nd > k || nd > bounds::kKsFusedMaxDigits)
+            return hipErrorInvalidValue;
+        for (int r = 0; r <= k; r++)
+            if (map.prime[r] == kSkipRow)
+                return hipErrorInvalidValue;
+        const KsMacSrc ks{ ext, ext_item, ext_digit, inb, inb_stride, key, key_comp, nd, k };
+        switch (e.logn)
+        {
+        case 14: return launch_half_inv<14>(e, prod, nrows, map, flags, nullptr, 0, nullptr, &ks);
+        case 15: return launch_half_inv<15>(e, prod, nrows, map, flags, nullptr, 0, nullptr, &ks);
+        case 16: return launch_half_inv<16>(e, prod, nrows, map, flags, nullptr, 0, nullptr, &ks);
         default: return hipErrorInvalidValue;
         }
     }
diff --git a/gemini-seal_amd/csrc/pipeline.cpp b/gemini-seal_amd/csrc/pipeline.cpp
--- a/gemini-seal_amd/csrc/pipeline.cpp
+++ b/gemini-seal_amd/csrc/pipeline.cpp
@@ -237,8 +237,16 @@
             return KsRows{ inb, inb_stride };
         }
 
+        struct KsMacOperands
+        {
+            KsRows in_bundle;
+            const u64 *ext;
+            std::size_t ext_digit;
+            const u64 *key;
+        };
         void ks_finish(Engine &e, LevelTools &lt, int k, u64 *prod, u64 *temp, u64 *ctp, std::size_t ct_stride, const u64 *c0p,
-                       std::size_t c0_stride, std::size_t m, unsigned *sink, bool one_component = false)
+                       std::size_t c0_stride, std::size_t m, unsigned *sink, bool one_component = false,
+                       const KsMacOperands *mac = nullptr)
         {
             const KsDev &h = lt.h_ks;
             const std::size_t N = e.n;
@@ -250,6 +258,8 @@
             u64 *const prod_rows = one_component ? prod - ext_item : prod;
             const std::size_t npolys = one_component ? m : 2 * m, prod_stride = one_component ? 2 * ext_item : ext_item;
             const int lead = one_component ? rows : 0;
+            if (mac && (ckks || one_component || !ks_mac_can_fuse(e, k)))
+                throw std::logic_error("internal: fused inner product misused");
             if (one_component)
             {
                 if (c0p || sink || ct_stride != 2 * static_cast<std::size_t>(k) * N || 2 * rows > kMaxRows)
@@ -264,9 +274,15 @@
             if (!ckks)
             {
                 const bool defer = ntt_can_defer_top(e, k);
-                check(launch_ntt(e, prod_rows, m * 2 * rows, map_rows, true, (defer ? kNttDeferTop : 0) | kNttAnyRep), "intt(prod)");
+                if (mac)
+                    check(launch_intt_ks_mac(e, h, prod, m, map_rows, mac->in_bundle.inb, mac->in_bundle.inb_stride, mac->ext, ext_item,
+                                             mac->ext_digit, mac->key),
+                          "intt(inner product)");
+                else
+                    check(launch_ntt(e, prod_rows, m * 2 * rows, map_rows, true, (defer ? kNttDeferTop : 0) | kNttAnyRep), "intt(prod)");
                 SinkArm arm(e, sink);
-                check(launch_ks_moddown_bfv(e, lt.d_ks, h, prod, prod_stride, ctp, ct_stride, npolys, defer, c0p, c0_stride),
+                check(launch_ks_moddown_bfv(e, lt.d_ks, h, prod, prod_stride, ctp, ct_stride, npolys, defer, c0p, c0_stride,
+                                            mac != nullptr),
                       "moddown_bfv");
                 return;
             }
@@ -377,6 +393,7 @@
         if (per_item != (w_coeff + w_ext + w_prod + w_temp) * sizeof(u64))
             throw std::logic_error("internal: arena accounting mismatch");
         const RowMap map_rows = lt.map_key;
+        const bool fuse_mac = !split && ks_mac_can_fuse(e, k);
         for_chunks(e, count, per_item, 4, [&](std::size_t off, std::size_t m) {
             u64 *coeff = w_coeff ? e.ws_alloc(w_coeff * m) : nullptr;
             u64 *ext = e.ws_alloc(w_ext * m);
@@ -397,6 +414,12 @@
             if (!finish)
             {
                 const KsRows in_bundle = ks_digits(e, lt, k, tg, target_stride, m, coeff, ext, dj0, dj1);
+                if (fuse_mac)
+                {
+                    const KsMacOperands mac{ in_bundle, ext, ext_digit, key.d_data };
+                    ks_finish(e, lt, k, prod, temp, ctp, ct_stride, c0p, c0_stride, m, sink_at(e, off), false, &mac);
+                    return;
+                }
                 check(launch_ks_mac(e, lt.d_ks, h, in_bundle.inb, in_bundle.inb_stride, ext, ext_item, ext_digit, key.d_data, prod,
                                     w_prod, m, dj0, dj1),
                       "mac");
```
